# LCSL/nys-koop-lqr

Measured on AMD Instinct MI355X. Metric: Nyström-Koopman fits/sec (K_nm build + A,B,C solve), N=1e5 m=2000 d=384, higher is better.
Workload: dtype f64

## Files before the change

### include/nyskoop.h

```cpp
#ifndef NYSKOOP_H
#define NYSKOOP_H

#include <stdint.h>

#ifdef __cplusplus
extern "C" {
#endif

#define NK_ABI_VERSION 2

enum {
  NK_OK = 0,
  NK_ERR_BAD_ARG = -1,
  NK_ERR_HIP = -2,
  NK_ERR_NOT_SPD = -3,
  NK_ERR_OOM = -4,
  NK_ERR_NO_CONVERGENCE = -5,
  NK_ERR_NO_DEVICE = -6
};

enum { NK_KERNEL_RBF = 0, NK_KERNEL_MATERN52 = 1, NK_KERNEL_LINEAR = 2, NK_KERNEL_TPS = 3 };

typedef struct nk_kernel_desc {
  int32_t type;
  int32_t d;
  int32_t n_lengthscale;
  int32_t reserved;
  const double* lengthscale;
  double sigma0;
} nk_kernel_desc;

typedef struct nk_fit_stats {
  double ms_total;
  double ms_upload;
  double ms_kmat;
  double ms_gram;
  double ms_sqrt;
  double ms_solve;
  double ms_gram_kernel_avg;
  int32_t gram_kernel_launches;
  int32_t sqrt_iters;
  double sqrt_residual;
  double gram_flops;
  double kmat_pairs;
  int32_t rank_inner;
  int32_t rank_inner_rec;
  double pivot_ratio_inner;
  double pivot_ratio_inner_rec;
  int32_t refined;
  int32_t reserved_;
  double refine_ratio_inner;
  double refine_ratio_inner_rec;
} nk_fit_stats;

typedef struct nk_ctx nk_ctx;
typedef struct nk_model nk_model;

int nk_version(void);
const char* nk_last_error(void);
int nk_device_count(void);
int nk_create(int device, nk_ctx** out);
int nk_destroy(nk_ctx* ctx);
int nk_synchronize(nk_ctx* ctx);
void* nk_stream(nk_ctx* ctx);
int nk_set_kmat_mode(nk_ctx* ctx, int mode);
int nk_set_strict_spd(nk_ctx* ctx, int strict);
int nk_set_refine(nk_ctx* ctx, double pivot_ratio, int32_t steps);
#define NK_DTYPE_F64 0
#define NK_DTYPE_F32 1
int nk_set_compute_dtype(nk_ctx* ctx, int dtype);
int nk_wait_stream(nk_ctx* ctx, void* producer_stream);
int nk_group_create(int device, int size, nk_ctx** members);
typedef struct nk_cv_unit {
  const nk_kernel_desc* kernel;
  double gamma;
  double jitter;
  int32_t m;
  int32_t reserved;
  int64_t test_begin, test_end;
  const int64_t* landmark_rows;
} nk_cv_unit;
int nk_cv_grid(nk_ctx* const* members, int32_t n_members, const double* X, int64_t ldx, const double* Y, int64_t ldy,
               int64_t n, int32_t d, int32_t p, const nk_cv_unit* units, int32_t n_units, double* scores, int32_t* status);
typedef struct nk_spline_cv_unit {
  double gamma;
  int32_t m;
  int32_t reserved;
  int64_t test_begin, test_end;
  const double* centers;
} nk_spline_cv_unit;
int nk_spline_cv_grid(nk_ctx* const* members, int32_t n_members, const double* X, int64_t ldx, const double* Y,
                      int64_t ldy, int64_t n, int32_t d, int32_t p, const nk_spline_cv_unit* units, int32_t n_units,
                      double* scores, int32_t* status);
int nk_group_enter(nk_ctx* member);
int nk_group_leave(nk_ctx* member);
int nk_group_stats(nk_ctx* member, uint64_t* out4);
int nk_runtime_counters(uint64_t* out, int32_t n);
int nk_shutdown(void);

void* nk_host_alloc(uint64_t bytes);
void nk_host_free(void* ptr);

int nk_kernel_matrix(nk_ctx* ctx, const nk_kernel_desc* kd,
                     const double* A, int64_t lda, int64_t nA,
                     const double* B, int64_t ldb, int64_t nB,
                     double* out, int64_t ldo);

int nk_nystrom_fit(nk_ctx* ctx, const nk_kernel_desc* kd,
                   const double* X, int64_t ldx, const double* Y, int64_t ldy,
                   int64_t n, int32_t d, int32_t p,
                   const int64_t* row_ranges, int32_t n_ranges,
                   const double* Zin, int64_t ldzi, const double* Zout, int64_t ldzo, int32_t m,
                   double gamma, double jitter,
                   nk_model** model, nk_fit_stats* stats);

int nk_gram_doubles(int32_t m, int32_t d, int32_t p, int64_t* count);
int nk_nystrom_gram(nk_ctx* ctx, const nk_kernel_desc* kd,
                    const double* X, int64_t ldx, const double* Y, int64_t ldy,
                    int64_t n, int32_t d, int32_t p,
                    const int64_t* row_ranges, int32_t n_ranges,
                    const double* Zin, int64_t ldzi, const double* Zout, int64_t ldzo, int32_t m,
                    double* gram, nk_fit_stats* stats);
int nk_nystrom_solve(nk_ctx* ctx, const nk_kernel_desc* kd,
                     const double* Zin, int64_t ldzi, const double* Zout, int64_t ldzo, int32_t m, int32_t d, int32_t p,
                     const double* gram, int64_t n_total, double gamma, double jitter,
                     nk_model** model, nk_fit_stats* stats);

int nk_model_create(nk_ctx* ctx, const nk_kernel_desc* kd, const double* Zout, int64_t ldz,
                    int32_t m, int32_t d, int32_t p, double jitter,
                    const double* A, const double* B, const double* C, const double* W,
                    nk_model** model);
int nk_model_destroy(nk_model* model);

int nk_spline_fit(nk_ctx* ctx, const double* X, int64_t ldx, const double* Y, int64_t ldy, int64_t n, int32_t d, int32_t p,
                  const int64_t* row_ranges, int32_t n_ranges, const double* centers, int64_t ldc, int32_t m, double gamma,
                  nk_model** model, nk_fit_stats* stats);
int nk_spline_model_create(nk_ctx* ctx, const double* centers, int64_t ldc, int32_t m, int32_t d, int32_t p,
                           const double* A, const double* B, const double* C, const double* W, nk_model** model);

int nk_model_get(nk_ctx* ctx, const nk_model* model, char which, double* out, int64_t ldo);
int nk_model_dims(const nk_model* model, int32_t* m, int32_t* d, int32_t* p);
int nk_model_get_ops(nk_ctx* ctx, const nk_model* model, double* G, int64_t ldg, double* C, int64_t ldc, double* W,
                     int64_t ldw);
int nk_model_get_ops_async(nk_ctx* ctx, nk_model* model, double* G, int64_t ldg, double* C, int64_t ldc, double* W,
                           int64_t ldw);
int nk_model_wait(nk_model* model);

int nk_lift(nk_ctx* ctx, const nk_model* model, const double* Xq, int64_t ldx, int64_t nq,
            double* out, int64_t ldo);

int nk_predict(nk_ctx* ctx, const nk_model* model, const double* Xaug, int64_t ldx, int64_t nq,
               double* out, int64_t ldo);

int nk_score_neg_rmse(nk_ctx* ctx, const nk_model* model, const double* Xaug, int64_t ldx,
                      const double* Ytrue, int64_t ldy, int64_t nq, double* score);

int nk_rollout(nk_ctx* ctx, const nk_model* model, const double* x0, int64_t ldx0,
               const double* U, int32_t T, int32_t batch, double* out_x, double* out_z);

int nk_closed_loop(nk_ctx* ctx, const nk_model* model, const double* K, const double* phi0,
                   const double* phi_ref, int32_t steps, double* out_x, double* out_u);
int nk_closed_loop_batch(nk_ctx* ctx, const nk_model* model, const double* K, const double* phi0,
                         const double* phi_ref, int32_t steps, int32_t batch, double* out_x, double* out_u);
#define NK_PLANT_DUFFING 0
#define NK_PLANT_DOUBLE_INTEGRATOR 1
#define NK_PLANT_HJB 2
int nk_plant_step(int plant, double Ts, const double* x, const double* u, double* x_next);
int nk_plant_loop(nk_ctx* ctx, const nk_model* model, int plant, double Ts, const double* K, const double* x0,
                  const double* x_ref, int32_t steps, int32_t batch, double* out_x, double* out_u);
int nk_linear_rollout(nk_ctx* ctx, const double* A, const double* B, const double* C, int32_t m, int32_t d, int32_t p,
                      const double* z0, const double* U, int32_t T, int32_t batch, double* out_x, double* out_z);

int nk_gemm_f32(nk_ctx* ctx, int64_t M, int64_t N, int64_t K, const float* A, int64_t lda, const float* B, int64_t ldb,
                double* C, int64_t ldc);
int nk_gemm(nk_ctx* ctx, int transA, int transB, int64_t M, int64_t N, int64_t K, double alpha,
            const double* A, int64_t lda, const double* B, int64_t ldb, double beta, double* C, int64_t ldc);
int nk_sqrtm_spd(nk_ctx* ctx, const double* P, int64_t ldp, int32_t m, double* S, double* Sinv,
                 int32_t* iters, double* residual);
int nk_solve_spd(nk_ctx* ctx, const double* P, int64_t ldp, int32_t m, const double* R, int64_t ldr,
                 int32_t nrhs, double* X, int64_t ldxo);

int nk_bench_gram(nk_ctx* ctx, int64_t n, int32_t m, int32_t p, int32_t d, int32_t reps, double* ms_avg, double* flop);

#define NK_CHOL_FLOW_GIVEUP (-0x40000000)
int nk_chol_aug(nk_ctx* ctx, int32_t nsys, const double* const* P, const int64_t* ldp, const int32_t* m,
                const double* const* R, const int32_t* extra, double* const* L, double* const* X, int32_t* failed,
                double* piv_ratio);

#ifdef __cplusplus
}
#endif
#endif
```

### nys_koop_lqr_amd/_lib.py

```python
import atexit
import ctypes as C
import os
import sys
import threading

import numpy as np

_HERE = os.path.dirname(os.path.abspath(__file__))

NK_KERNEL_RBF, NK_KERNEL_MATERN52, NK_KERNEL_LINEAR, NK_KERNEL_TPS = 0, 1, 2, 3
NK_PLANT_DUFFING, NK_PLANT_DOUBLE_INTEGRATOR, NK_PLANT_HJB = 0, 1, 2
NK_OK = 0
_ERR_NAMES = {-1: "NK_ERR_BAD_ARG", -2: "NK_ERR_HIP", -3: "NK_ERR_NOT_SPD", -4: "NK_ERR_OOM",
              -5: "NK_ERR_NO_CONVERGENCE", -6: "NK_ERR_NO_DEVICE"}


class NyskoopError(RuntimeError):
    def __init__(self, code, msg):
        super().__init__(f"{_ERR_NAMES.get(code, code)}: {msg}")
        self.code = code


class KernelDesc(C.Structure):
    _fields_ = [("type", C.c_int32), ("d", C.c_int32), ("n_lengthscale", C.c_int32), ("reserved", C.c_int32),
                ("lengthscale", C.POINTER(C.c_double)), ("sigma0", C.c_double)]


class CvUnit(C.Structure):
    _fields_ = [("kernel", C.POINTER(KernelDesc)), ("gamma", C.c_double), ("jitter", C.c_double), ("m", C.c_int32),
                ("reserved", C.c_int32), ("test_begin", C.c_int64), ("test_end", C.c_int64),
                ("landmark_rows", C.POINTER(C.c_int64))]


class SplineCvUnit(C.Structure):
    _fields_ = [("gamma", C.c_double), ("m", C.c_int32), ("reserved", C.c_int32), ("test_begin", C.c_int64),
                ("test_end", C.c_int64), ("centers", C.POINTER(C.c_double))]


class FitStats(C.Structure):
    _fields_ = [("ms_total", C.c_double), ("ms_upload", C.c_double), ("ms_kmat", C.c_double),
                ("ms_gram", C.c_double), ("ms_sqrt", C.c_double), ("ms_solve", C.c_double),
                ("ms_gram_kernel_avg", C.c_double), ("gram_kernel_launches", C.c_int32),
                ("sqrt_iters", C.c_int32), ("sqrt_residual", C.c_double), ("gram_flops", C.c_double),
                ("kmat_pairs", C.c_double), ("rank_inner", C.c_int32), ("rank_inner_rec", C.c_int32),
                ("pivot_ratio_inner", C.c_double), ("pivot_ratio_inner_rec", C.c_double), ("refined", C.c_int32),
                ("reserved_", C.c_int32), ("refine_ratio_inner", C.c_double), ("refine_ratio_inner_rec", C.c_double)]

    def as_dict(self):
        return {k: getattr(self, k) for k, _ in self._fields_}


_P = C.c_void_p
_I64 = C.c_int64
_I32 = C.c_int32
_D = C.c_double

SIGNATURES = {
    "nk_version": (C.c_int, []),
    "nk_last_error": (C.c_char_p, []),
    "nk_device_count": (C.c_int, []),
    "nk_create": (C.c_int, [C.c_int, C.POINTER(_P)]),
    "nk_destroy": (C.c_int, [_P]),
    "nk_synchronize": (C.c_int, [_P]),
    "nk_stream": (_P, [_P]),
    "nk_set_kmat_mode": (C.c_int, [_P, C.c_int]),
    "nk_set_strict_spd": (C.c_int, [_P, C.c_int]),
    "nk_set_refine": (C.c_int, [_P, C.c_double, C.c_int32]),
    "nk_wait_stream": (C.c_int, [_P, _P]),
    "nk_shutdown": (C.c_int, []),
    "nk_group_create": (C.c_int, [C.c_int, C.c_int, C.POINTER(_P)]),
    "nk_group_enter": (C.c_int, [_P]),
    "nk_group_leave": (C.c_int, [_P]),
    "nk_set_compute_dtype": (C.c_int, [_P, C.c_int]),
    "nk_group_stats": (C.c_int, [_P, C.POINTER(C.c_uint64)]),
    "nk_runtime_counters": (C.c_int, [C.POINTER(C.c_uint64), C.c_int32]),
    "nk_cv_grid": (C.c_int, [C.POINTER(_P), _I32, _P, _I64, _P, _I64, _I64, _I32, _I32, C.POINTER(CvUnit), _I32,
                             C.POINTER(_D), C.POINTER(_I32)]),
    "nk_spline_cv_grid": (C.c_int, [C.POINTER(_P), _I32, _P, _I64, _P, _I64, _I64, _I32, _I32, C.POINTER(SplineCvUnit),
                                    _I32, C.POINTER(_D), C.POINTER(_I32)]),
    "nk_host_alloc": (_P, [C.c_uint64]),
    "nk_host_free": (None, [_P]),
    "nk_kernel_matrix": (C.c_int, [_P, C.POINTER(KernelDesc), _P, _I64, _I64, _P, _I64, _I64, _P, _I64]),
    "nk_nystrom_fit": (C.c_int, [_P, C.POINTER(KernelDesc), _P, _I64, _P, _I64, _I64, _I32, _I32,
                                 C.POINTER(_I64), _I32, _P, _I64, _P, _I64, _I32, _D, _D,
                                 C.POINTER(_P), C.POINTER(FitStats)]),
    "nk_gram_doubles": (C.c_int, [_I32, _I32, _I32, C.POINTER(_I64)]),
    "nk_nystrom_gram": (C.c_int, [_P, C.POINTER(KernelDesc), _P, _I64, _P, _I64, _I64, _I32, _I32,
                                  C.POINTER(_I64), _I32, _P, _I64, _P, _I64, _I32, _P, C.POINTER(FitStats)]),
    "nk_nystrom_solve": (C.c_int, [_P, C.POINTER(KernelDesc), _P, _I64, _P, _I64, _I32, _I32, _I32, _P, _I64, _D, _D,
                                   C.POINTER(_P), C.POINTER(FitStats)]),
    "nk_model_create": (C.c_int, [_P, C.POINTER(KernelDesc), _P, _I64, _I32, _I32, _I32, _D, _P, _P, _P, _P,
                                  C.POINTER(_P)]),
    "nk_spline_fit": (C.c_int, [_P, _P, _I64, _P, _I64, _I64, _I32, _I32, C.POINTER(_I64), _I32, _P, _I64, _I32, _D,
                                C.POINTER(_P), C.POINTER(FitStats)]),
    "nk_spline_model_create": (C.c_int, [_P, _P, _I64, _I32, _I32, _I32, _P, _P, _P, _P, C.POINTER(_P)]),
    "nk_model_destroy": (C.c_int, [_P]),
    "nk_model_get": (C.c_int, [_P, _P, C.c_char, _P, _I64]),
    "nk_model_dims": (C.c_int, [_P, C.POINTER(_I32), C.POINTER(_I32), C.POINTER(_I32)]),
    "nk_model_get_ops": (C.c_int, [_P, _P, _P, _I64, _P, _I64, _P, _I64]),
    "nk_model_get_ops_async": (C.c_int, [_P, _P, _P, _I64, _P, _I64, _P, _I64]),
    "nk_model_wait": (C.c_int, [_P]),
    "nk_lift": (C.c_int, [_P, _P, _P, _I64, _I64, _P, _I64]),
    "nk_predict": (C.c_int, [_P, _P, _P, _I64, _I64, _P, _I64]),
    "nk_score_neg_rmse": (C.c_int, [_P, _P, _P, _I64, _P, _I64, _I64, C.POINTER(_D)]),
    "nk_rollout": (C.c_int, [_P, _P, _P, _I64, _P, _I32, _I32, _P, _P]),
    "nk_closed_loop": (C.c_int, [_P, _P, _P, _P, _P, _I32, _P, _P]),
    "nk_closed_loop_batch": (C.c_int, [_P, _P, _P, _P, _P, _I32, _I32, _P, _P]),
    "nk_plant_step": (C.c_int, [C.c_int, _D, _P, _P, _P]),
    "nk_plant_loop": (C.c_int, [_P, _P, C.c_int, _D, _P, _P, _P, _I32, _I32, _P, _P]),
    "nk_linear_rollout": (C.c_int, [_P, _P, _P, _P, _I32, _I32, _I32, _P, _P, _I32, _I32, _P, _P]),
    "nk_gemm_f32": (C.c_int, [_P, _I64, _I64, _I64, _P, _I64, _P, _I64, _P, _I64]),
    "nk_gemm": (C.c_int, [_P, C.c_int, C.c_int, _I64, _I64, _I64, _D, _P, _I64, _P, _I64, _D, _P, _I64]),
    "nk_sqrtm_spd": (C.c_int, [_P, _P, _I64, _I32, _P, _P, C.POINTER(_I32), C.POINTER(_D)]),
    "nk_solve_spd": (C.c_int, [_P, _P, _I64, _I32, _P, _I64, _I32, _P, _I64]),
    "nk_bench_gram": (C.c_int, [_P, _I64, _I32, _I32, _I32, _I32, C.POINTER(_D), C.POINTER(_D)]),
    "nk_chol_aug": (C.c_int, [_P, _I32, _P, _P, _P, _P, _P, _P, _P, _P, _P]),
}

_lib = None
_lib_lock = threading.Lock()


def library_path():
    return os.environ.get("NYSKOOP_LIB", os.path.join(_HERE, "libnyskoop.so"))


def load_library():
    global _lib
    with _lib_lock:
        if _lib is None:
            path = library_path()
            if not os.path.exists(path):
                raise NyskoopError(-6, f"{path} not found: build it with `python -c 'import __graft_entry__ as g; "
                                       f"g.build()'` or `make -C nys_koop_lqr_amd/csrc` (there is no CPU fallback)")
            if os.environ.get("NYSKOOP_PRELOAD_TORCH", "1") == "1" and "torch" not in sys.modules:
                try:
                    import torch
                except Exception:
                    pass
            lib = C.CDLL(path)
            for name, (res, args) in SIGNATURES.items():
                fn = getattr(lib, name)
                fn.restype = res
                fn.argtypes = args
            _lib = lib
            atexit.register(shutdown)
    return _lib


def shutdown():
    lib = _lib
    if lib is None:
        return
    with _pools_lock:
        pools = list(_pools.values())
        _pools.clear()
        lpools = list(_lockstep_pools.values())
        _lockstep_pools.clear()
    for pool in pools:
        pool.shutdown(wait=True)
    for pool in lpools:
        pool.close()
    _PinnedBlock.drain()
    lib.nk_shutdown()


def check(rc):
    if rc != NK_OK:
        raise NyskoopError(rc, load_library().nk_last_error().decode("utf-8", "replace"))


def runtime_counters():
    v = (C.c_uint64 * 5)()
    check(load_library().nk_runtime_counters(v, 5))
    return dict(chain_giveups=int(v[0]), jacobi_giveups=int(v[1]), rank_truncated_fits=int(v[2]), sqrt_retries=int(v[3]),
                refined_fits=int(v[4]))


def torch_if_cuda():
    try:
        import torch
    except Exception:
        return None
    try:
        return torch if torch.cuda.is_available() else None
    except Exception:
        return None


class Mat:

    def __init__(self, obj, rows=None, cols=None):
        if hasattr(obj, "data_ptr") and hasattr(obj, "stride"):
            if str(getattr(obj, "dtype", "")).split(".")[-1] not in ("float64", "double"):
                raise TypeError("device tensors must be float64")
            if obj.dim() != 2 or (obj.shape[1] > 1 and obj.stride(1) != 1):
                raise ValueError("device tensors must be 2-D with unit inner stride")
            self.owner, self.ptr, self.ld = obj, obj.data_ptr(), int(obj.stride(0))
            self.shape = (int(obj.shape[0]), int(obj.shape[1]))
        else:
            a = np.asarray(obj, dtype=np.float64)
            if a.ndim == 1:
                a = a.reshape(1, -1)
            if a.ndim != 2:
                raise ValueError("expected a 2-D array")
            if a.shape[1] > 0 and a.shape[0] > 0 and (a.strides[1] != 8 or a.strides[0] % 8 or a.strides[0] < 8 * a.shape[1]):
                a = np.ascontiguousarray(a)
            self.owner, self.ptr = a, a.ctypes.data
            self.ld = a.strides[0] // 8 if a.shape[0] > 1 else max(a.shape[1], 1)
            self.shape = a.shape
        if self.shape[0] <= 1:
            self.ld = max(self.ld, self.shape[1], 1)
        if rows is not None and self.shape[0] != rows or cols is not None and self.shape[1] != cols:
            raise ValueError(f"expected a {rows} x {cols} matrix, got {self.shape}")


class Context:

    def __init__(self, device=0, handle=None):
        self.lib = load_library()
        if handle is None:
            handle = _P()
            check(self.lib.nk_create(int(device), C.byref(handle)))
        self.handle = handle
        self.device = int(device)

    def enter(self):
        check(self.lib.nk_group_enter(self.handle))

    def leave(self):
        check(self.lib.nk_group_leave(self.handle))

    def close(self):
        if getattr(self, "handle", None):
            self.lib.nk_destroy(self.handle)
# ... 268 lines not shown
```

### nys_koop_lqr_amd/csrc/nk_api.hip

```cpp
#include "nk_common.h"
#include "nk_plant.h"

#include <cmath>
#include <cstdarg>
#include <cstdio>
#include <cstring>
#include <chrono>
#include <cstdlib>
#include <algorithm>
#include <condition_variable>
#include <functional>
#include <mutex>
#include <set>
#include <thread>

namespace nk {

static thread_local std::string g_err;

void set_error(const char* fmt, ...) {
  char buf[1024];
  va_list ap;
  va_start(ap, fmt);
  vsnprintf(buf, sizeof(buf), fmt, ap);
// ... 197 lines not shown
    if (g_pool[i].device == device && g_pool[i].bytes == bytes) {
      double* p = g_pool[i].ptr;
      g_pool.erase(g_pool.begin() + i);
      return p;
    }
  return nullptr;
}
static void pool_give(int device, size_t bytes, double* ptr) {
  {
    std::lock_guard<std::mutex> lk(g_pool_mu);
    if (g_pool.size() < 512) {
      g_pool.push_back(ModelBuf{device, bytes, ptr});
      return;
    }
  }
  (void)hipSetDevice(device);
  (void)hipFree(ptr);
}
static void pool_drain() {
  std::lock_guard<std::mutex> lk(g_pool_mu);
  for (auto& b : g_pool) {
    (void)hipSetDevice(b.device);
    (void)hipFree(b.ptr);
  }
  g_pool.clear();
}

static int model_alloc(nk_ctx* ctx, int m, int d, int p, nk_model** out, int kind = NK_MODEL_NYSTROM) {
  nk_model* mdl = new nk_model();
  mdl->device = ctx->device;
  mdl->m = m; mdl->d = d; mdl->p = p;
  mdl->kind = kind;
  const size_t mp = (size_t)m + p;
  const size_t nS = kind == NK_MODEL_SPLINE ? 0 : 2 * (size_t)m * m;
  const size_t total = (size_t)m * mp  + (size_t)d * m  + (size_t)d * mp  + nS +
                       (size_t)m * d  + (size_t)d  + 64;
  mdl->bytes = total * sizeof(double);
  mdl->buf = pool_take(ctx->device, mdl->bytes);
  if (!mdl->buf) {
    hipError_t e = hipMalloc(reinterpret_cast<void**>(&mdl->buf), mdl->bytes);
    if (e != hipSuccess) {
      (void)hipGetLastError();
      delete mdl;
      set_error("model allocation of %zu bytes failed: %s", total * sizeof(double), hipGetErrorString(e));
      return NK_ERR_OOM;
    }
  }
  double* q = mdl->buf;
  auto take = [&](size_t cnt) { double* r = q; q += (cnt + 1) & ~(size_t)1; return r; };
  mdl->A = take((size_t)m * mp);
  mdl->B = mdl->A + m;
  mdl->C = take((size_t)d * m);
  mdl->W = take((size_t)d * mp);
  if (kind != NK_MODEL_SPLINE) {
    mdl->S = take((size_t)m * m);
    mdl->Sinv = take((size_t)m * m);
  }
  mdl->Z = take((size_t)m * d);
  mdl->winv = take((size_t)d);
  {
    std::lock_guard<std::mutex> lk(g_reg_mu);
    g_models.insert(mdl);
  }
  *out = mdl;
  return NK_OK;
}

static int lift_device(nk_ctx* ctx, const nk_model* mdl, const double* Xq, int64_t ldx, int64_t nq, double* out,
                       int64_t ldo) {
  const int m = mdl->m;
  if (mdl->kind == NK_MODEL_SPLINE)
    return launch_kmat(ctx, mdl->ktype, Xq, ldx, nq, mdl->Z, mdl->d, m, mdl->d, mdl->winv, mdl->sigma0, out, ldo);
  const int64_t chunk = 32768;
  const ArenaMark mk = arena_mark(ctx);
  double* Kq = nullptr;
  NK_TRY(arena_alloc_t(ctx, (size_t)(nq < chunk ? nq : chunk) * m, &Kq));
  for (int64_t r0 = 0; r0 < nq; r0 += chunk) {
    const int64_t len = nq - r0 < chunk ? nq - r0 : chunk;
    NK_TRY(launch_kmat(ctx, mdl->ktype, Xq + r0 * ldx, ldx, len, mdl->Z, mdl->d, m, mdl->d, mdl->winv, mdl->sigma0, Kq,
                       m));
    NK_TRY(launch_gemm(ctx, false, false, len, m, m, 1.0, Kq, m, mdl->Sinv, m, 0.0, out + r0 * ldo, ldo));
  }
  arena_release(ctx, mk);
  return NK_OK;
}

static int predict_device(nk_ctx* ctx, const nk_model* mdl, const double* Xaug, int64_t ldx, int64_t nq, double* out,
                          int64_t ldo) {
  const int m = mdl->m, d = mdl->d, p = mdl->p;
  const int64_t chunk = 32768;
  const ArenaMark mk = arena_mark(ctx);
  double* phi = nullptr;
  NK_TRY(arena_alloc_t(ctx, (size_t)(nq < chunk ? nq : chunk) * m, &phi));
  for (int64_t r0 = 0; r0 < nq; r0 += chunk) {
    const int64_t len = nq - r0 < chunk ? nq - r0 : chunk;
    NK_TRY(lift_device(ctx, mdl, Xaug + r0 * ldx, ldx, len, phi, m));
    NK_TRY(launch_gemm(ctx, false, true, len, d, m, 1.0, phi, m, mdl->W, m + p, 0.0, out + r0 * ldo, ldo));
    if (p > 0)
      NK_TRY(launch_gemm(ctx, false, true, len, d, p, 1.0, Xaug + r0 * ldx + d, ldx, mdl->W + m, m + p, 1.0,
                         out + r0 * ldo, ldo));
  }
  arena_release(ctx, mk);
  return NK_OK;
}

struct HostTrace {
  bool on;
  std::chrono::steady_clock::time_point t0, last;
  HostTrace() : on(getenv("NYSKOOP_TRACE") != nullptr) { t0 = last = std::chrono::steady_clock::now(); }
  void mark(const char* what) {
    if (!on) return;
    auto now = std::chrono::steady_clock::now();
    fprintf(stderr, "[nk trace] %-28s +%8.3f ms (total %8.3f)\n", what,
            std::chrono::duration<double, std::milli>(now - last).count(),
            std::chrono::duration<double, std::milli>(now - t0).count());
    last = now;
  }
};

static float ev_ms(nk_ctx* ctx, int a, int b) {
  float ms = 0.f;
  (void)hipEventElapsedTime(&ms, ctx->ev[a], ctx->ev[b]);
  return ms;
}

}

using namespace nk;

extern "C" {

int nk_version(void) { return NK_ABI_VERSION; }

const char* nk_last_error(void) { return g_err.c_str(); }

int nk_device_count(void) {
  int n = 0;
  if (hipGetDeviceCount(&n) != hipSuccess) {
    (void)hipGetLastError();
    return 0;
  }
  return n;
}

int nk_create(int device, nk_ctx** out) {
  NK_REQUIRE(out != nullptr, "nk_create: null output pointer");
  *out = nullptr;
  int n = nk_device_count();
  if (n <= 0) {
    set_error("no HIP device visible: libnyskoop has no CPU fallback");
    return NK_ERR_NO_DEVICE;
  }
  NK_REQUIRE(device >= 0 && device < n, "nk_create: device %d out of range (0..%d)", device, n - 1);
  NK_HIP(hipSetDevice(device));
  hipDeviceProp_t prop;
  NK_HIP(hipGetDeviceProperties(&prop, device));
  if (strncmp(prop.gcnArchName, "gfx950", 6) != 0) {
    set_error("device %d is %s; libnyskoop is built for gfx950 (MI355X) only", device, prop.gcnArchName);
    return NK_ERR_NO_DEVICE;
  }
  nk_ctx* ctx = new nk_ctx();
  ctx->device = device;
  ctx->num_cu = prop.multiProcessorCount;
  int prio_lo = 0, prio_hi = 0;
  NK_HIP(hipDeviceGetStreamPriorityRange(&prio_lo, &prio_hi));
  const int prio_mid = (prio_lo - prio_hi >= 2) ? (prio_lo + prio_hi) / 2 : prio_hi;
  NK_HIP(hipStreamCreateWithPriority(&ctx->stream_main, hipStreamNonBlocking, prio_mid));
  NK_HIP(hipStreamCreateWithPriority(&ctx->stream_side, hipStreamNonBlocking, prio_lo));
  NK_HIP(hipStreamCreateWithPriority(&ctx->stream_prep, hipStreamNonBlocking, prio_hi));
  NK_HIP(hipStreamCreateWithFlags(&ctx->stream_copy, hipStreamNonBlocking));
  NK_HIP(hipStreamCreateWithPriority(&ctx->stream_la[0], hipStreamNonBlocking, prio_hi));
  NK_HIP(hipStreamCreateWithPriority(&ctx->stream_la[1], hipStreamNonBlocking, prio_mid));
  for (int q = 0; q < 2; ++q)
    for (int i = 0; i < 4; ++i) NK_HIP(hipEventCreateWithFlags(&ctx->ev_la[q][i], hipEventDisableTiming));
  ctx->stream = ctx->stream_main;
  ctx->cur_arena = &ctx->arena;
  NK_HIP(hipEventCreateWithFlags(&ctx->ev_fork, hipEventDisableTiming));
  NK_HIP(hipEventCreateWithFlags(&ctx->ev_join, hipEventDisableTiming));
  NK_HIP(hipEventCreateWithFlags(&ctx->ev_chain, hipEventDisableTiming));
  NK_HIP(hipMalloc(reinterpret_cast<void**>(&ctx->d_info), 256));
  ctx->d_piv = reinterpret_cast<unsigned long long*>(ctx->d_info + 16);
  NK_HIP(hipMalloc(reinterpret_cast<void**>(&ctx->d_scalars), 64 * sizeof(double)));
  NK_HIP(hipHostMalloc(reinterpret_cast<void**>(&ctx->h_scalars), 64 * sizeof(double), hipHostMallocMapped | hipHostMallocCoherent));
  NK_HIP(hipHostMalloc(reinterpret_cast<void**>(&ctx->h_info), 256, hipHostMallocMapped | hipHostMallocCoherent));
  ctx->h_piv = reinterpret_cast<unsigned long long*>(ctx->h_info + 16);
  for (int i = 0; i < 16; ++i) NK_HIP(hipEventCreate(&ctx->ev[i]));
  NK_HIP(hipEventCreateWithFlags(&ctx->ev_ext, hipEventDisableTiming));
  for (int i = 0; i < 8; ++i) NK_HIP(hipEventCreateWithFlags(&ctx->ev_up[i], hipEventDisableTiming));
  const char* km = getenv("NYSKOOP_KMAT");
  ctx->kmat_mode = (km && strcmp(km, "direct") == 0) ? 1 : 0;
  const char* st = getenv("NYSKOOP_STRICT_SPD");
  ctx->strict_spd = (st && atoi(st) != 0) ? 1 : 0;
  if (const char* rp = getenv("NYSKOOP_REFINE_PIVOT")) ctx->refine_pivot = atof(rp);
  if (const char* rs = getenv("NYSKOOP_REFINE_STEPS")) ctx->refine_steps = std::max(0, atoi(rs));
  {
    std::lock_guard<std::mutex> lk(g_reg_mu);
    g_ctxs.insert(ctx);
  }
  *out = ctx;
  return NK_OK;
}

static void destroy_ctx_unregistered(nk_ctx* ctx) {
  (void)hipSetDevice(ctx->device);
  if (tl_ctx == ctx) tl_ctx = nullptr;
  group_detach(ctx);
  (void)hipStreamSynchronize(ctx->stream_main);
  (void)hipStreamSynchronize(ctx->stream_side);
  (void)hipStreamSynchronize(ctx->stream_prep);
  (void)hipStreamSynchronize(ctx->stream_copy);
  for (int q = 0; q < 2; ++q) {
    if (ctx->stream_la[q]) { (void)hipStreamSynchronize(ctx->stream_la[q]); (void)hipStreamDestroy(ctx->stream_la[q]); }
    for (int i = 0; i < 4; ++i) if (ctx->ev_la[q][i]) (void)hipEventDestroy(ctx->ev_la[q][i]);
  }
  for (auto& c : ctx->arena.chunks) (void)hipFree(c.base);
  for (auto& c : ctx->arena_side.chunks) (void)hipFree(c.base);
  (void)hipEventDestroy(ctx->ev_fork);
  (void)hipEventDestroy(ctx->ev_join);
  if (ctx->ev_chain) (void)hipEventDestroy(ctx->ev_chain);
  if (ctx->ev_ext) (void)hipEventDestroy(ctx->ev_ext);
  for (int i = 0; i < 8; ++i) if (ctx->ev_up[i]) (void)hipEventDestroy(ctx->ev_up[i]);
  (void)hipStreamDestroy(ctx->stream_side);
  (void)hipStreamDestroy(ctx->stream_prep);
  (void)hipStreamDestroy(ctx->stream_copy);
  (void)hipFree(ctx->d_info);
  for (int i = 0; i < 2; ++i) if (ctx->d_flow[i]) (void)hipFree(ctx->d_flow[i]);
  (void)hipFree(ctx->d_scalars);
  if (ctx->d_zeros) (void)hipFree(ctx->d_zeros);
  if (ctx->h_stage) (void)hipHostFree(ctx->h_stage);
  (void)hipHostFree(ctx->h_scalars);
  (void)hipHostFree(ctx->h_info);
  for (int i = 0; i < 16; ++i) (void)hipEventDestroy(ctx->ev[i]);
  (void)hipStreamDestroy(ctx->stream_main);
  delete ctx;
}

int nk_destroy(nk_ctx* ctx) {
  if (!ctx) return NK_OK;
  {
    std::lock_guard<std::mutex> lk(g_reg_mu);
    if (g_ctxs.erase(ctx) == 0) return NK_OK;
  }
  destroy_ctx_unregistered(ctx);
  return NK_OK;
}

static int model_wait_unchecked(nk_model* mdl);
static void destroy_model_unregistered(nk_model* model, bool to_pool) {
  (void)model_wait_unchecked(model);
  if (to_pool) {
    pool_give(model->device, model->bytes, model->buf);
  } else {
    (void)hipSetDevice(model->device);
    (void)hipFree(model->buf);
  }
  delete model;
}

int nk_shutdown(void) {
  tl_ctx = nullptr;
  std::set<nk_ctx*> ctxs;
  std::set<nk_model*> models;
  std::set<void*> blocks;
  {
    std::lock_guard<std::mutex> lk(g_reg_mu);
    ctxs.swap(g_ctxs);
    models.swap(g_models);
    blocks.swap(g_host_blocks);
  }
  for (nk_ctx* c : ctxs) {
    (void)hipSetDevice(c->device);
    (void)hipStreamSynchronize(c->stream_main);
    (void)hipStreamSynchronize(c->stream_side);
    (void)hipStreamSynchronize(c->stream_prep);
    (void)hipStreamSynchronize(c->stream_copy);
  }
  for (nk_model* m : models) destroy_model_unregistered(m, false);
  for (nk_ctx* c : ctxs) destroy_ctx_unregistered(c);
  pool_drain();
  for (void* b : blocks) (void)hipHostFree(b);
  return NK_OK;
}

int nk_set_compute_dtype(nk_ctx* ctx, int dtype) {
  NK_REQUIRE(ctx != nullptr && (dtype == NK_DTYPE_F64 || dtype == NK_DTYPE_F32), "nk_set_compute_dtype: bad argument");
  ctx->compute_f32 = dtype == NK_DTYPE_F32 ? 1 : 0;
  return NK_OK;
}

int nk_set_strict_spd(nk_ctx* ctx, int strict) {
  NK_REQUIRE(ctx != nullptr && strict >= 0 && strict <= 2, "nk_set_strict_spd: bad argument");
  ctx->strict_spd = strict;
  return NK_OK;
}

int nk_set_refine(nk_ctx* ctx, double pivot_ratio, int32_t steps) {
  NK_REQUIRE(ctx != nullptr && pivot_ratio >= 0.0 && pivot_ratio <= 1.0 && steps >= 0 && steps <= 8, "nk_set_refine: bad argument");
  ctx->refine_pivot = pivot_ratio;
  ctx->refine_steps = steps;
  return NK_OK;
}

int nk_wait_stream(nk_ctx* ctx, void* producer_stream) {
  NK_REQUIRE(ctx != nullptr, "nk_wait_stream: null context");
  NK_HIP(hipSetDevice(ctx->device));
  if (ctx->group) {
    hipError_t e = real_stream_sync(reinterpret_cast<hipStream_t>(producer_stream));
    if (e != hipSuccess) { set_error("synchronising the producer stream failed: %s", hipGetErrorString(e)); return NK_ERR_HIP; }
    return NK_OK;
  }
  NK_HIP(hipEventRecord(ctx->ev_ext, reinterpret_cast<hipStream_t>(producer_stream)));
  NK_HIP(hipStreamWaitEvent(ctx->stream_main, ctx->ev_ext, 0));
  NK_HIP(hipStreamWaitEvent(ctx->stream_side, ctx->ev_ext, 0));
  NK_HIP(hipStreamWaitEvent(ctx->stream_prep, ctx->ev_ext, 0));
  NK_HIP(hipStreamWaitEvent(ctx->stream_copy, ctx->ev_ext, 0));
  return NK_OK;
}

int nk_group_create(int device, int size, nk_ctx** out) {
  NK_REQUIRE(out != nullptr && size >= 1 && size <= 256, "nk_group_create: bad argument");
  for (int i = 0; i < size; ++i) out[i] = nullptr;
  for (int i = 0; i < size; ++i) {
    int rc = nk_create(device, &out[i]);
    if (rc != NK_OK) {
      for (int j = 0; j < i; ++j) { nk_destroy(out[j]); out[j] = nullptr; }
      return rc;
    }
  }
  nk_group* g = group_new(device, size);
  if (!g) {
    for (int i = 0; i < size; ++i) { nk_destroy(out[i]); out[i] = nullptr; }
    set_error("nk_group_create: could not create the shared stream / argument table");
    return NK_ERR_HIP;
  }
  for (int i = 0; i < size; ++i) group_attach(g, i, out[i]);
  return NK_OK;
}

int nk_group_enter(nk_ctx* ctx) {
  NK_REQUIRE(ctx != nullptr, "nk_group_enter: null context");
  return group_enter(ctx);
}

// ... 125 lines not shown
  for (int k = 0; k < B; ++k) set_phase(members[k], k, 1);
  run_units(all, true);
  for (int k = 0; k < B; ++k) set_phase(members[k], k, 0);
  const auto t_mid = std::chrono::steady_clock::now();
  if (!deferred.empty()) {
    std::sort(deferred.begin(), deferred.end());
    for (int k = 0; k < B; ++k) set_phase(members[k], k, 2);
    run_units(deferred, false);
    for (int k = 0; k < B; ++k) set_phase(members[k], k, 0);
  }
  if (cv_trace)
    fprintf(stderr, "[nyskoop] %s: %d units in %.3f s, %zu rank-deficient units again in %.3f s (%d members)\n", what, n_units,
            std::chrono::duration<double>(t_mid - t_start).count(), deferred.size(),
            std::chrono::duration<double>(std::chrono::steady_clock::now() - t_mid).count(), B);
  return NK_OK;
}

int nk_cv_grid(nk_ctx* const* members, int32_t n_members, const double* X, int64_t ldx, const double* Y, int64_t ldy,
               int64_t n, int32_t d, int32_t p, const nk_cv_unit* units, int32_t n_units, double* scores, int32_t* status) {
  NK_REQUIRE(members && n_members >= 1 && X && Y && units && scores, "nk_cv_grid: null argument");
  NK_REQUIRE(n > 0 && d > 0 && p >= 0 && n_units >= 0 && ldx >= d + p && ldy >= d, "nk_cv_grid: bad sizes");
  for (int k = 0; k < n_members; ++k) NK_REQUIRE(members[k] != nullptr, "nk_cv_grid: null member context");
  for (int u = 0; u < n_units; ++u) {
    const nk_cv_unit& cu = units[u];
    NK_REQUIRE(cu.kernel && cu.landmark_rows && cu.m > 0, "nk_cv_grid: unit %d: null kernel / landmarks", u);
    NK_REQUIRE(0 <= cu.test_begin && cu.test_begin < cu.test_end && cu.test_end <= n, "nk_cv_grid: unit %d: bad test fold", u);
    for (int j = 0; j < cu.m; ++j)
      NK_REQUIRE(cu.landmark_rows[j] >= 0 && cu.landmark_rows[j] < n, "nk_cv_grid: unit %d: landmark row out of range", u);
  }
  auto fit_score = [&](nk_ctx* ctx, int u, const CvData& dt, std::vector<double>& Z, double* sc) -> int {
    const nk_cv_unit& cu = units[u];
    Z.resize((size_t)cu.m * d);
    for (int j = 0; j < cu.m; ++j) memcpy(&Z[(size_t)j * d], dt.Yh + cu.landmark_rows[j] * dt.ldyh, (size_t)d * 8);
    const int64_t rr[4] = {0, cu.test_begin, cu.test_end, n};
    nk_model* mdl = nullptr;
    int rc = nk_nystrom_fit(ctx, cu.kernel, dt.Xd, dt.ldxd, dt.Yd, dt.ldyd, n, d, p, rr, 2, nullptr, 0, Z.data(), d, cu.m,
                            cu.gamma, cu.jitter, &mdl, nullptr);
    if (rc == NK_OK)
      rc = nk_score_neg_rmse(ctx, mdl, dt.Xd + cu.test_begin * dt.ldxd, dt.ldxd, dt.Yd + cu.test_begin * dt.ldyd, dt.ldyd,
                             cu.test_end - cu.test_begin, sc);
    if (mdl) nk_model_destroy(mdl);
    return rc;
  };
  std::vector<int> saved_strict((size_t)n_members);
  for (int k = 0; k < n_members; ++k) saved_strict[(size_t)k] = members[k]->strict_spd;
  auto set_phase = [&](nk_ctx* ctx, int k, int phase) {
    ctx->strict_spd = phase == 1 ? 1 : (phase == 2 ? 0 : saved_strict[(size_t)k]);
  };
  return cv_grid_run("cv_grid", members, n_members, X, ldx, Y, ldy, n, d, p, n_units, true, fit_score, set_phase, scores,
                     status);
}

int nk_spline_cv_grid(nk_ctx* const* members, int32_t n_members, const double* X, int64_t ldx, const double* Y, int64_t ldy,
                      int64_t n, int32_t d, int32_t p, const nk_spline_cv_unit* units, int32_t n_units, double* scores,
                      int32_t* status) {
  NK_REQUIRE(members && n_members >= 1 && X && Y && units && scores, "nk_spline_cv_grid: null argument");
  NK_REQUIRE(n > 0 && d > 0 && p >= 0 && n_units >= 0 && ldx >= d + p && ldy >= d, "nk_spline_cv_grid: bad sizes");
  for (int k = 0; k < n_members; ++k) NK_REQUIRE(members[k] != nullptr, "nk_spline_cv_grid: null member context");
  for (int u = 0; u < n_units; ++u) {
    const nk_spline_cv_unit& cu = units[u];
    NK_REQUIRE(cu.centers && cu.m > 0, "nk_spline_cv_grid: unit %d: null centres / m <= 0", u);
    NK_REQUIRE(!is_device_ptr(cu.centers), "nk_spline_cv_grid: unit %d: centres must be a host pointer", u);
    NK_REQUIRE(0 <= cu.test_begin && cu.test_begin < cu.test_end && cu.test_end <= n,
               "nk_spline_cv_grid: unit %d: bad test fold", u);
  }
  auto fit_score = [&](nk_ctx* ctx, int u, const CvData& dt, std::vector<double>&, double* sc) -> int {
    const nk_spline_cv_unit& cu = units[u];
    const int64_t rr[4] = {0, cu.test_begin, cu.test_end, n};
    nk_model* mdl = nullptr;
    int rc = nk_spline_fit(ctx, dt.Xd, dt.ldxd, dt.Yd, dt.ldyd, n, d, p, rr, 2, cu.centers, d, cu.m, cu.gamma, &mdl, nullptr);
    if (rc == NK_OK)
      rc = nk_score_neg_rmse(ctx, mdl, dt.Xd + cu.test_begin * dt.ldxd, dt.ldxd, dt.Yd + cu.test_begin * dt.ldyd, dt.ldyd,
                             cu.test_end - cu.test_begin, sc);
    if (mdl) nk_model_destroy(mdl);
    return rc;
  };
  auto set_phase = [&](nk_ctx* ctx, int, int phase) { ctx->spline_defer_svd = phase == 1; };
  return cv_grid_run("spline_cv_grid", members, n_members, X, ldx, Y, ldy, n, d, p, n_units, false, fit_score, set_phase,
                     scores, status);
}

int nk_synchronize(nk_ctx* ctx) {
  NK_REQUIRE(ctx != nullptr, "null context");
  tl_ctx = ctx;
  NK_HIP(hipStreamSynchronize(ctx->stream));
  return NK_OK;
}

void* nk_stream(nk_ctx* ctx) { return ctx ? reinterpret_cast<void*>(ctx->stream) : nullptr; }

void* nk_host_alloc(uint64_t bytes) {
  void* p = nullptr;
  if (hipHostMalloc(&p, bytes ? bytes : 1, hipHostMallocDefault) != hipSuccess) {
    (void)hipGetLastError();
    set_error("hipHostMalloc of %llu bytes failed", (unsigned long long)bytes);
    return nullptr;
  }
  std::lock_guard<std::mutex> lk(g_reg_mu);
  g_host_blocks.insert(p);
  return p;
}

void nk_host_free(void* ptr) {
  if (!ptr) return;
  {
    std::lock_guard<std::mutex> lk(g_reg_mu);
    if (g_host_blocks.erase(ptr) == 0) return;
  }
  (void)hipHostFree(ptr);
}

int nk_set_kmat_mode(nk_ctx* ctx, int mode) {
  NK_REQUIRE(ctx != nullptr && (mode == 0 || mode == 1), "nk_set_kmat_mode: bad argument");
  ctx->kmat_mode = mode;
  return NK_OK;
}

int nk_kernel_matrix(nk_ctx* ctx, const nk_kernel_desc* kd, const double* A, int64_t lda, int64_t nA, const double* B,
                     int64_t ldb, int64_t nB, double* out, int64_t ldo) {
  NK_TRY(check_ctx(ctx));
  NK_REQUIRE(kd && A && B && out, "nk_kernel_matrix: null argument");
  NK_REQUIRE(nA >= 0 && nB >= 0 && kd->d > 0, "nk_kernel_matrix: negative size");
  NK_REQUIRE(lda >= kd->d && ldb >= kd->d && ldo >= nB, "nk_kernel_matrix: leading dimension too small");
  if (nA == 0 || nB == 0) return NK_OK;
  const int d = kd->d;
  double* winv = nullptr;
  NK_TRY(arena_alloc_t(ctx, (size_t)d, &winv));
  NK_TRY(make_winv(ctx, kd, d, winv));
  MatIn a, b;
  NK_TRY(stage_in(ctx, A, lda, nA, d, &a));
  NK_TRY(stage_in(ctx, B, ldb, nB, d, &b));
  MatOut o;
  NK_TRY(stage_out(ctx, out, ldo, nA, nB, &o));
  if (kd->type == NK_KERNEL_TPS && ctx->kmat_mode == 0 && d >= 32 && nA >= 2 && nB >= 2) {
    const int64_t lta = (nA + 1) & ~(int64_t)1, ltb = (nB + 1) & ~(int64_t)1;
    double *center = nullptr, *At = nullptr, *sqa = nullptr, *Bt = nullptr, *sqb = nullptr;
    NK_TRY(arena_alloc_t(ctx, (size_t)d, &center));
    NK_TRY(arena_alloc_t(ctx, (size_t)d * lta, &At));
    NK_TRY(arena_alloc_t(ctx, (size_t)nA, &sqa));
    NK_TRY(arena_alloc_t(ctx, (size_t)d * ltb, &Bt));
    NK_TRY(arena_alloc_t(ctx, (size_t)nB, &sqb));
    NK_TRY(launch_colmean(ctx, b.ptr, b.ld, (int)nB, d, center));
    NK_TRY(prep_rows(ctx, a.ptr, a.ld, nA, d, winv, center, At, lta, sqa));
    NK_TRY(prep_rows(ctx, b.ptr, b.ld, nB, d, winv, center, Bt, ltb, sqb));
    NK_TRY(launch_kmat_gram(ctx, NK_KERNEL_TPS, At, lta, sqa, nA, Bt, ltb, sqb, nB, d, 0.0, o.dev, o.ld));
  } else {
    NK_TRY(launch_kmat(ctx, kd->type, a.ptr, a.ld, nA, b.ptr, b.ld, nB, d, winv, kd->sigma0, o.dev, o.ld));
  }
  NK_TRY(finish_out(ctx, o));
  NK_HIP(hipStreamSynchronize(ctx->stream));
  return NK_OK;
}

static inline size_t gram_block1(int m, int p) { return (((size_t)(2 * m + p) * (m + p)) + 1) & ~(size_t)1; }
static inline size_t gram_doubles(int m, int d, int p) { return gram_block1(m, p) + (size_t)(m + d) * m; }

enum { FIT_FULL = 0, FIT_GRAM = 1, FIT_SOLVE = 2 };

static int fit_impl(nk_ctx* ctx, const nk_kernel_desc* kd, const double* X, int64_t ldx, const double* Y, int64_t ldy,
                    int64_t n, int32_t d, int32_t p, const int64_t* row_ranges, int32_t n_ranges, const double* Zin,
                    int64_t ldzi, const double* Zout, int64_t ldzo, int32_t m, double gamma, double jitter,
                    nk_model** model, nk_fit_stats* stats, int mode, double* gram_io) {
  HostTrace tr;
  NK_TRY(check_ctx(ctx));
  tr.mark("check_ctx/arena_reset");
  NK_REQUIRE(kd && Zout, "nk_nystrom_fit: null argument");
  NK_REQUIRE(mode == FIT_SOLVE || (X && Y), "nk_nystrom_fit: null data pointer");
  NK_REQUIRE(mode == FIT_GRAM || model != nullptr, "nk_nystrom_fit: null model pointer");
  NK_REQUIRE(mode == FIT_FULL || gram_io != nullptr, "nk_nystrom_gram/solve: null accumulator");
  NK_REQUIRE(n > 0 && d > 0 && p >= 0 && m > 0, "nk_nystrom_fit: sizes must be positive (n=%lld d=%d p=%d m=%d)",
             (long long)n, d, p, m);
  NK_REQUIRE(mode == FIT_SOLVE || (ldx >= d + p && ldy >= d), "nk_nystrom_fit: leading dimension too small");
  NK_REQUIRE(ldzo >= d, "nk_nystrom_fit: leading dimension too small");
  NK_REQUIRE(std::isfinite(gamma) && std::isfinite(jitter), "nk_nystrom_fit: gamma/jitter not finite");
  NK_REQUIRE(kd->type != NK_KERNEL_TPS, "nk_nystrom_fit: the thin-plate spline has no Nystrom fit (nk_spline_fit)");
  if (model) *model = nullptr;
  std::vector<int64_t> rng;
  if (mode != FIT_SOLVE && row_ranges && n_ranges > 0) {
    for (int i = 0; i < n_ranges; ++i) {
      const int64_t b = row_ranges[2 * i], e = row_ranges[2 * i + 1];
      NK_REQUIRE(0 <= b && b <= e && e <= n, "nk_nystrom_fit: row range %d = [%lld,%lld) outside [0,%lld)", i,
                 (long long)b, (long long)e, (long long)n);
      if (e > b) { rng.push_back(b); rng.push_back(e); }
    }
  } else {
    rng.push_back(0); rng.push_back(n);
  }
  int64_t n_eff = 0;
  for (size_t i = 0; i < rng.size(); i += 2) n_eff += rng[i + 1] - rng[i];
  NK_REQUIRE(n_eff > 0, "nk_nystrom_fit: no training rows selected");
  const bool same_centers = (Zin == nullptr) || (Zin == Zout && ldzi == ldzo);
  const int mp = m + p;
  const double gamma_n = gamma * (double)n_eff;

  nk_model* mdl = nullptr;
  NK_TRY(model_alloc(ctx, m, d, p, &mdl));
  struct Guard {
    nk_ctx* c;
    nk_model* m;
    ~Guard() {
      if (m) {
        (void)hipStreamSynchronize(c->stream_main);
        (void)hipStreamSynchronize(c->stream_side);
        (void)hipStreamSynchronize(c->stream_prep);
        (void)hipStreamSynchronize(c->stream_la[0]);
        (void)hipStreamSynchronize(c->stream_la[1]);
        nk_model_destroy(m);
      }
    }
  } guard{ctx, mdl};
  mdl->ktype = kd->type; mdl->sigma0 = kd->sigma0; mdl->jitter = jitter;

  tr.mark("validate + model_alloc");
  hipEvent_t* ev = ctx->ev;
  NK_HIP(hipEventRecord(ev[0], ctx->stream));
  NK_TRY(make_winv(ctx, kd, d, mdl->winv));
  MatIn x, y, zi, zo;
  int host_passes = 1;
  if (mode != FIT_SOLVE) {
    const char* e = getenv("NYSKOOP_HOST_PASSES");
    const int want = e ? atoi(e) : 6;
    if (want > 1 && rng.size() == 2 && !ctx_recording(ctx) && (double)n_eff * (2.0 * d + p) * 8.0 >= 64e6 &&
        !is_device_ptr(X) && !is_device_ptr(Y))
      host_passes = want > 8 ? 8 : want;
  }
  if (mode != FIT_SOLVE && host_passes > 1) {
    x.ld = (d + p + 1) & ~(int64_t)1;
    y.ld = (d + 1) & ~(int64_t)1;
    double *xd = nullptr, *yd = nullptr;
    NK_TRY(arena_alloc_t(ctx, (size_t)n * x.ld, &xd));
    NK_TRY(arena_alloc_t(ctx, (size_t)n * y.ld, &yd));
    x.ptr = xd; y.ptr = yd; x.staged = y.staged = true;
  } else if (mode != FIT_SOLVE) {
    NK_TRY(stage_in(ctx, X, ldx, n, d + p, &x));
    NK_TRY(stage_in(ctx, Y, ldy, n, d, &y));
  }
  if (mode != FIT_SOLVE && rng.size() > 2 && (double)n_eff * (2.0 * d + p) * 8.0 <= 256e6) {
    const int64_t ldxg = (d + p + 1) & ~(int64_t)1, ldyg = (d + 1) & ~(int64_t)1;
    double *xg = nullptr, *yg = nullptr;
    NK_TRY(arena_alloc_t(ctx, (size_t)n_eff * ldxg, &xg));
    NK_TRY(arena_alloc_t(ctx, (size_t)n_eff * ldyg, &yg));
    int64_t o = 0;
    for (size_t i = 0; i < rng.size(); i += 2) {
      const int64_t b = rng[i], len = rng[i + 1] - rng[i];
      NK_TRY(launch_copy2d(ctx, x.ptr + b * x.ld, x.ld, xg + o * ldxg, ldxg, len, d + p));
      NK_TRY(launch_copy2d(ctx, y.ptr + b * y.ld, y.ld, yg + o * ldyg, ldyg, len, d));
      o += len;
    }
    x.ptr = xg; x.ld = ldxg; y.ptr = yg; y.ld = ldyg;
    rng.assign({(int64_t)0, n_eff});
  }
  NK_TRY(stage_in(ctx, Zout, ldzo, m, d, &zo));
  if (same_centers) zi = zo; else NK_TRY(stage_in(ctx, Zin, ldzi, m, d, &zi));
  NK_TRY(launch_copy2d(ctx, zo.ptr, zo.ld, mdl->Z, d, m, d));
  NK_HIP(hipEventRecord(ev[1], ctx->stream));
  tr.mark("staging issued");

  double *Kmm = nullptr, *Kj = nullptr, *Kj_in = nullptr, *Kxo = nullptr;
  bool landmarks_aside = false;
  if (mode != FIT_GRAM) {
  NK_TRY(arena_alloc_t(ctx, (size_t)m * m, &Kmm));
  NK_TRY(arena_alloc_t(ctx, (size_t)m * m, &Kj));
  if (same_centers) {
    Kj_in = Kj;
    Kxo = Kmm;
  } else {
    NK_TRY(arena_alloc_t(ctx, (size_t)m * m, &Kj_in));
    NK_TRY(arena_alloc_t(ctx, (size_t)m * m, &Kxo));
  }
  {
    const char* la = getenv("NYSKOOP_LANDMARKS_ASIDE");
    landmarks_aside = mode == FIT_FULL && n_eff >= 20000 && m >= 1024 && !ctx_recording(ctx) && !(la && la[0] == '0');
  }
  {
    hipStream_t s0 = ctx->stream;
    if (landmarks_aside) {
      NK_HIP(hipEventRecord(ev[12], ctx->stream));
      ctx->stream = ctx->stream_prep;
      NK_HIP(hipStreamWaitEvent(ctx->stream, ev[12], 0));
    }
    int rc_l = launch_kmat(ctx, kd->type, zo.ptr, zo.ld, m, zo.ptr, zo.ld, m, d, mdl->winv, kd->sigma0, Kmm, m);
    if (rc_l == NK_OK) rc_l = launch_copy2d(ctx, Kmm, m, Kj, m, m, m);
    if (rc_l == NK_OK) rc_l = launch_add_diag(ctx, Kj, m, m, jitter);
    if (rc_l == NK_OK && !same_centers) {
      rc_l = launch_kmat(ctx, kd->type, zi.ptr, zi.ld, m, zi.ptr, zi.ld, m, d, mdl->winv, kd->sigma0, Kj_in, m);
      if (rc_l == NK_OK) rc_l = launch_add_diag(ctx, Kj_in, m, m, jitter);
      if (rc_l == NK_OK) rc_l = launch_kmat(ctx, kd->type, zi.ptr, zi.ld, m, zo.ptr, zo.ld, m, d, mdl->winv, kd->sigma0, Kxo, m);
    }
    const hipError_t he = rc_l == NK_OK ? hipEventRecord(ev[8], ctx->stream) : hipSuccess;
    ctx->stream = s0;
    NK_TRY(rc_l);
    NK_HIP(he);
  }
  }
  double *G1 = nullptr, *G2 = nullptr, *G3 = nullptr, *G4 = nullptr;
  const int64_t ldd = d + (d & 1);
  NK_TRY(arena_alloc_t(ctx, gram_doubles(m, d, p), &G1));
  G2 = G1 + (size_t)mp * mp;
  G3 = G1 + gram_block1(m, p);
  G4 = G3 + (size_t)m * m;
  float ms_gram_kernel = 0.f;
  int gram_launches = 0;
  bool gram_deferred = false;
  const bool timed = stats != nullptr;
  SqrtPlan splan;
  int it = 0;
// ... 1640 lines not shown
```

### nys_koop_lqr_amd/csrc/nk_common.h

```cpp
#pragma once
#include <hip/hip_runtime.h>
#include <stdint.h>
#include <stddef.h>
#include <string>
#include <vector>

#include "nyskoop.h"
#include "nk_lockstep.h"

namespace nk {

void set_error(const char* fmt, ...);

#define NK_HIP(call)                                                                         \
  do {                                                                                       \
    hipError_t e_ = (call);                                                                  \
    if (e_ != hipSuccess) {                                                                  \
      nk::set_error("%s failed: %s (%s:%d)", #call, hipGetErrorString(e_), __FILE__, __LINE__); \
      return e_ == hipErrorOutOfMemory ? NK_ERR_OOM : NK_ERR_HIP;                            \
    }                                                                                        \
  } while (0)

#define NK_TRY(call)            \
  do {                          \
    int rc_ = (call);           \
    if (rc_ != NK_OK) return rc_; \
  } while (0)

#define NK_REQUIRE(cond, ...)     \
  do {                            \
    if (!(cond)) {                \
      nk::set_error(__VA_ARGS__); \
      return NK_ERR_BAD_ARG;      \
    }                             \
  } while (0)

struct ArenaChunk {
  char* base = nullptr;
  size_t cap = 0;
  size_t off = 0;
};
struct Arena {
  std::vector<ArenaChunk> chunks;
  int cur = 0;
};
struct ArenaMark {
  int chunk;
  size_t off;
};

}

struct nk_member_state;
struct nk_ctx {
  int device = 0;
  hipStream_t stream = nullptr;
  hipStream_t stream_main = nullptr;
  hipStream_t stream_side = nullptr;
  hipStream_t stream_copy = nullptr;
  hipStream_t stream_prep = nullptr;
  nk::Arena arena;
  nk::Arena arena_side;
  nk::Arena* cur_arena = nullptr;
  hipStream_t stream_la[2] = {nullptr, nullptr};
  hipEvent_t ev_la[2][4] = {};
  int compute_f32 = 0;
  hipEvent_t ev_fork = nullptr, ev_join = nullptr, ev_chain = nullptr;
  int* d_info = nullptr;
  unsigned long long* d_piv = nullptr;
  unsigned long long* h_piv = nullptr;
  double* d_scalars = nullptr;
  double* h_scalars = nullptr;
  int* h_info = nullptr;
  double* d_zeros = nullptr;
  hipEvent_t ev[16];
  int num_cu = 256;
  int kmat_mode = 0;
  double refine_pivot = 0.0;
  int refine_steps = 2;
  int strict_spd = 0;
  hipEvent_t ev_ext = nullptr;
  hipEvent_t ev_up[8] = {};
  nk_group* group = nullptr;
  nk_member_state* gstate = nullptr;
  int* d_flow[2] = {nullptr, nullptr};
  size_t flow_words[2] = {0, 0};
  bool spline_defer_svd = false;
  bool chol_flow_off = false;
  double* h_stage = nullptr;
  size_t h_stage_bytes = 0;
};

enum { NK_MODEL_NYSTROM = 0, NK_MODEL_SPLINE = 1 };
struct nk_model {
  int device = 0;
  int32_t m = 0, d = 0, p = 0;
  int32_t ktype = 0;
  double sigma0 = 0.0;
  double jitter = 0.0;
  double* buf = nullptr;
  size_t bytes = 0;
  double *A = nullptr, *B = nullptr, *C = nullptr, *W = nullptr, *S = nullptr, *Sinv = nullptr, *Z = nullptr,
         *winv = nullptr;
  bool has_ops = false;
  int32_t kind = 0;
  hipEvent_t ev_fetch = nullptr;
};

namespace nk {

struct SideScope {
  nk_ctx* c;
  hipStream_t s0;
  Arena* a0;
  explicit SideScope(nk_ctx* ctx, hipStream_t s = nullptr) : c(ctx), s0(ctx->stream), a0(ctx->cur_arena) {
    c->stream = s ? s : c->stream_side;
    c->cur_arena = &c->arena_side;
  }
  ~SideScope() {
    c->stream = s0;
    c->cur_arena = a0;
  }
};

struct ChainOnly {
  nk_ctx* c;
  bool b0;
  explicit ChainOnly(nk_ctx* ctx) : c(ctx), b0(ctx->chol_flow_off) { c->chol_flow_off = true; }
  ~ChainOnly() { c->chol_flow_off = b0; }
};

inline int info_base(const nk_ctx* c) { return c->stream != c->stream_main ? 2 : 0; }

__device__ __forceinline__ double exp_nonpos_ca() {
  double ca = __longlong_as_double(0x3e5ade156a5dcb37LL);
  asm volatile("" : "+v"(ca));
  return ca;
}
__device__ __forceinline__ double exp_nonpos(double x, double ca_v) {
  const double k = __builtin_rint(x * __longlong_as_double(0x3ff71547652b82feLL));
  double r = __builtin_fma(__longlong_as_double((long long)0xbfe62e42fefa39efULL), k, x);
  r = __builtin_fma(__longlong_as_double((long long)0xbc7abc9e3b39803fULL), k, r);
  double p;
#define NK_EXP_STEP(c) asm("v_fma_f64 %0, %1, %2, %3" : "=v"(p) : "v"(r), "v"(p), "s"(c))
  asm("v_fma_f64 %0, %1, %2, %3" : "=v"(p) : "v"(r), "v"(ca_v), "s"(__longlong_as_double(0x3e928af3fca7ab0cLL)));
  NK_EXP_STEP(__longlong_as_double(0x3ec71dee623fde64LL));
  NK_EXP_STEP(__longlong_as_double(0x3efa01997c89e6b0LL));
  NK_EXP_STEP(__longlong_as_double(0x3f2a01a014761f6eLL));
  NK_EXP_STEP(__longlong_as_double(0x3f56c16c1852b7b0LL));
  NK_EXP_STEP(__longlong_as_double(0x3f81111111122322LL));
  NK_EXP_STEP(__longlong_as_double(0x3fa55555555502a1LL));
  NK_EXP_STEP(__longlong_as_double(0x3fc5555555555511LL));
  NK_EXP_STEP(__longlong_as_double(0x3fe000000000000bLL));
#undef NK_EXP_STEP
  p = __builtin_fma(r, p, 1.0);
  p = __builtin_fma(r, p, 1.0);
  return x < -1075.0 ? 0.0 : ldexp(p, (int)k);
}
__device__ __forceinline__ double exp_nonpos(double x) { return exp_nonpos(x, exp_nonpos_ca()); }

__host__ __device__ __forceinline__ double log_pos(double x) {
#pragma clang fp contract(off)
  const double ln2_hi = 6.93147180369123816490e-01, ln2_lo = 1.90821492927058770002e-10;
  const double Lg1 = 6.666666666666735130e-01, Lg2 = 3.999999999940941908e-01, Lg3 = 2.857142874366239149e-01,
               Lg4 = 2.222219843214978396e-01, Lg5 = 1.818357216161805012e-01, Lg6 = 1.531383769920937332e-01,
               Lg7 = 1.479819860511658591e-01;
  uint64_t bits;
  __builtin_memcpy(&bits, &x, 8);
  int32_t hx = (int32_t)(bits >> 32);
  int k = 0;
  if (hx < 0x00100000) {
    x *= 1.80143985094819840000e+16;
    k -= 54;
    __builtin_memcpy(&bits, &x, 8);
    hx = (int32_t)(bits >> 32);
  }
  k += (hx >> 20) - 1023;
  hx &= 0x000fffff;
  const int32_t i = (hx + 0x95f64) & 0x100000;
  bits = ((uint64_t)(uint32_t)(hx | (i ^ 0x3ff00000)) << 32) | (bits & 0xffffffffULL);
  __builtin_memcpy(&x, &bits, 8);
  k += i >> 20;
  const double f = x - 1.0;
  const double dk = (double)k;
  if ((0x000fffff & (2 + hx)) < 3) {
    if (f == 0.0) return k == 0 ? 0.0 : dk * ln2_hi + dk * ln2_lo;
    const double R = f * f * (0.5 - 0.33333333333333333 * f);
    return k == 0 ? f - R : dk * ln2_hi - ((R - dk * ln2_lo) - f);
  }
  const double s = f / (2.0 + f);
  const double z = s * s;
  const double w = z * z;
  const double t1 = w * (Lg2 + w * (Lg4 + w * Lg6));
  const double t2 = z * (Lg1 + w * (Lg3 + w * (Lg5 + w * Lg7)));
  const double R = t2 + t1;
  if (((hx - 0x6147a) | (0x6b851 - hx)) > 0) {
    const double hfsq = 0.5 * f * f;
    return k == 0 ? f - (hfsq - s * (hfsq + R)) : dk * ln2_hi - ((hfsq - (s * (hfsq + R) + dk * ln2_lo)) - f);
  }
  return k == 0 ? f - s * (f - R) : dk * ln2_hi - ((s * (f - R) - dk * ln2_lo) - f);
}
__host__ __device__ __forceinline__ double tps_value(double r2) {
#pragma clang fp contract(off)
  return r2 > 0.0 ? r2 * log_pos(sqrt(r2)) : 0.0;
}

nk_group* group_new(int device, int size);
void group_attach(nk_group* g, int slot, nk_ctx* c);
void group_detach(nk_ctx* c);
int group_enter(nk_ctx* c);
int group_leave(nk_ctx* c);
void group_stats(nk_ctx* c, uint64_t out[4]);
enum { CNT_CHAIN_GIVEUP = 0, CNT_JACOBI_GIVEUP = 1, CNT_RANK_TRUNCATED = 2, CNT_SQRT_RETRY = 3, CNT_REFINED = 4,
       CNT_CHOL_FLOW_GIVEUP = 5, CNT_CHOL_FLOW = 6, CNT_N = 7 };
void count_event(int which);
uint64_t read_counter(int which);
hipError_t real_stream_sync(hipStream_t s);
hipError_t real_event_sync(hipEvent_t e);

int arena_reset(nk_ctx* ctx);
ArenaMark arena_mark(nk_ctx* ctx);
void arena_release(nk_ctx* ctx, ArenaMark mk);
int arena_alloc(nk_ctx* ctx, size_t bytes, void** out);
template <typename T>
inline int arena_alloc_t(nk_ctx* ctx, size_t count, T** out) {
  return arena_alloc(ctx, count * sizeof(T), reinterpret_cast<void**>(out));
}
bool is_device_ptr(const void* p);

int launch_kmat(nk_ctx* ctx, int ktype, const double* A, int64_t lda, int64_t nA, const double* B, int64_t ldb,
                int64_t nB, int d, const double* winv, double sigma0, double* out, int64_t ldo);

enum { TRI_FULL = 0, TRI_UPPER_MIRROR = 1, TRI_LOWER = 2 };
struct GemmOpts {
  int tri = TRI_FULL;
  int splitk = 0;
};
int launch_gemm(nk_ctx* ctx, bool transA, bool transB, int64_t M, int64_t N, int64_t K, double alpha, const double* A,
                int64_t lda, const double* B, int64_t ldb, double beta, double* C, int64_t ldc,
                const GemmOpts& opts = GemmOpts(), float* ms_kernel = nullptr);

struct GemmCall {
  int64_t M = 0, N = 0, K = 0;
  double alpha = 1.0, beta = 0.0;
  const double* A = nullptr;
  const double* B = nullptr;
  double* C = nullptr;
  int64_t lda = 0, ldb = 0, ldc = 0;
  GemmOpts opts;
};
int launch_gemm_pair(nk_ctx* ctx, bool transA, bool transB, const GemmCall* calls, int ncalls);

struct TnSkip;
int launch_add_diag(nk_ctx* ctx, double* A, int64_t lda, int n, double v);
int launch_copy2d(nk_ctx* ctx, const double* src, int64_t lds, double* dst, int64_t ldd, int64_t rows, int64_t cols);
int launch_axpby2d(nk_ctx* ctx, double a, const double* X, int64_t ldx, double b, double* Y, int64_t ldy,
                   int64_t rows, int64_t cols);
int launch_scale_add_identity(nk_ctx* ctx, double a, const double* X, int64_t ldx, double c, double* Y, int64_t ldy,
                              int n, const TnSkip* skip = nullptr);
int launch_fill(nk_ctx* ctx, double* A, int64_t lda, int64_t rows, int64_t cols, double v);
int launch_frob_minus_identity(nk_ctx* ctx, const double* M, int64_t ldm, int n, double* d_out,
                               const TnSkip* skip = nullptr);
int launch_max_abs_rowsum(nk_ctx* ctx, const double* M, int64_t ldm, int n, double* d_out);
int launch_colsum_sqdiff(nk_ctx* ctx, const double* P, int64_t ldp, const double* Y, int64_t ldy, int64_t rows,
                         int cols, double* d_colsum);

int sqrtm_spd(nk_ctx* ctx, const double* P, int64_t ldp, int m, double* S, double* Sinv, int* iters, double* resid);
struct SqrtPlan {
  const double* P = nullptr;
  int64_t ldp = 0;
  int m = 0;
  double* W = nullptr;
  double* Linv = nullptr;
  double* X0 = nullptr;
  double* X0t = nullptr;
  double* d_sc = nullptr;
  ArenaMark mark{0, 0};
  bool deferred = false;
  int rc = 0, iters = 0, kmax = 0;
  double resid = 0.0;
  double lambda_min_hint = 0.0;
  bool early = false;
  int info_slot = 2;
  bool flow_gave_up = false;
  hipEvent_t pause_event = nullptr;
  int pause_step = -1;
};
constexpr int NK_SQRT_RETRY = 1;
int sqrtm_spd_coupled(nk_ctx* ctx, const double* P, int64_t ldp, int m, double* S, double* Sinv, int* iters, double* resid);
int sqrtm_prepare(nk_ctx* ctx, const double* P, int64_t ldp, int m, SqrtPlan* plan);
int sqrtm_finish(nk_ctx* ctx, SqrtPlan* plan, double* S, double* Sinv);
int sqrtm_verdict(nk_ctx* ctx, SqrtPlan* plan, int* iters, double* resid);
int cholesky_lower(nk_ctx* ctx, double* P, int64_t ldp, int m, double* Linv );
int cholesky_solve(nk_ctx* ctx, const double* L, int64_t ldl, int m, const double* Linv, double* R, int64_t ldr,
                   int nrhs);
struct CholSys {
  double* P = nullptr;
  int64_t ldp = 0;
  int m = 0;
  int extra = 0;
  bool backward = true;
  double* Linv = nullptr;
  double* pivlog = nullptr;
  double* R = nullptr;
  int64_t ldr = 0;
  int nrhs = 0;
};
int cholesky_lower_pair(nk_ctx* ctx, const CholSys* sys, int nsys);
int cholesky_lower_pair_async(nk_ctx* ctx, const CholSys* sys, int nsys);
int cholesky_check_pair(nk_ctx* ctx, const CholSys* sys, int nsys);
int cholesky_solve_pair(nk_ctx* ctx, const CholSys* sys, int nsys);
int cholesky_aug_pair_async(nk_ctx* ctx, const CholSys* sys, int nsys, hipEvent_t pause = nullptr, int pause_step = -1);
constexpr int CHOL_NB = 64;
constexpr int CHOL_WS = 2 * CHOL_NB * CHOL_NB + 8;
constexpr double CHOL_FIX_KAPPA = 8.0 * CHOL_NB;
inline int chol_fix_enabled() {
  const char* e = getenv("NYSKOOP_CHOL_FIX");
  return (e && e[0] == '0') ? 0 : ((e && e[0] == '2') ? 2 : 1);
}
bool launch_chol_trail_pair(nk_ctx* ctx, const GemmCall* calls, int ncalls, int* rc);
bool launch_chol_trail_potrf_pair(nk_ctx* ctx, const GemmCall* calls, int ncalls, const int* nb, double* const* Linv, int blk,
                                  double* const* plog, int* rc);
inline bool chol_fuse_enabled() {
  const char* e = getenv("NYSKOOP_CHOL_FUSE");
  return !(e && e[0] == '0');
}
bool chol_flow_enabled();
int cholesky_flow_pair(nk_ctx* ctx, const CholSys* sys, int nsys);
constexpr int CHOL_FLOW_GIVEUP = -0x40000000;
bool launch_chol_panel_pair(nk_ctx* ctx, const GemmCall* calls, int ncalls, int* rc);
int launch_trsm_right_lower_pair(nk_ctx* ctx, const CholSys* sys, int nsys);

struct PinvInfo {
  int rank = 0, sweeps = 0;
  bool converged = false;
  double sigma_max = 0.0, sigma_min_kept = 0.0, sigma_min = 0.0;
};
int pinv_right_divide(nk_ctx* ctx, const double* P, int64_t ldp, int m, const double* E, int64_t lde, int rows,
                      double* E_out, int64_t ldeo, double rcond, PinvInfo* info);
int cholesky_fail_flags(nk_ctx* ctx, const CholSys* sys, int nsys, int* failed , double* piv_ratio = nullptr);

int launch_lifted_step(nk_ctx* ctx, const double* G, int64_t ldg, int m, int mz, int pu, const double* z, int64_t zstride,
                       const double* u, int64_t ustride, const double* bias, double* out, int64_t ostride, int batch);

struct ChainArgs {
  const double* G = nullptr; int64_t ldg = 0; int m = 0, pu = 0;
  const double* z0 = nullptr; int64_t z0_stride = 0;
  bool lift = false;
  const double* x0 = nullptr; int64_t x0_stride = 0;
  const double* Zl = nullptr; int d = 0; const double* winv = nullptr; const double* Sinv = nullptr; int ktype = 0;
  double sigma0 = 0.0;
  const double* U = nullptr; int64_t u_stride = 0;
  const double* bias = nullptr; int64_t bias_stride = 0;
  double* Zall = nullptr; int64_t z_stride = 0;
  int T = 0, batch = 0;
};
int launch_ref_minus_traj(nk_ctx* ctx, const double* ref, int64_t ref_stride, const double* Phi, int64_t phi_stride,
                          double* D, int64_t d_stride, int steps, int m, int batch);
bool lifted_chain_ok(int m, int pu, int d_lift);
int launch_lifted_chain(nk_ctx* ctx, const ChainArgs& a);
bool lifted_chain_mw_ok(const nk_ctx* ctx, int m, int pu);
int chain_mw_workgroups(int m);
int chain_mw_group(int m, int batch);
int launch_lifted_chain_mw(nk_ctx* ctx, const ChainArgs& a);
int lifted_chain_mw_reset(nk_ctx* ctx);
int lifted_chain_mw_fetch_status(nk_ctx* ctx);
bool lifted_chain_mw_timed_out(nk_ctx* ctx, int* row, int* step, int* traj);
// ... 113 lines not shown
```

### nys_koop_lqr_amd/csrc/nk_gemm_tn.hip

```cpp
#include "nk_common.h"
#include "nk_tn_kstep.inc"
#include "nk_tn_shared.h"

#include <cstdlib>
#include <cstring>

namespace nk {

typedef double d4 __attribute__((ext_vector_type(4)));

constexpr int TBK = 16;
constexpr int TSTRIDE = 144;
constexpr int TSTAGE = 2 * TBK * TSTRIDE;
constexpr int TN_LDS_BYTES = 2 * TSTAGE * 8;

struct TnDev {
  const double* A;
  const double* B;
  int64_t lda, ldb;
  int M, N;
  int tiles_n;
  int tri;
  int ktrim;
  int tile_begin;
  double* C;
  int64_t ldc;
  double alpha, beta;
  double* Ct;
  int64_t ldct;
  const double* A_even;
  const double* B_even;
  double* Caff;
  double aff_a, aff_c;
};
struct TnParams {
  TnDev p[TN_MAXP];
  int nprob;
  int ntiles;
  int K, splitk, klen;
  int kmask;
  int use_asm;
  const double* zeros;
  double* slab;
  const double* skip_state;
  int skip_step;
  const double* select_state;
  const double* sqa;
  const double* sqb;
  double* out;
  int64_t ldo;
  int ktype;
  double sigma0sq;
};

__device__ __forceinline__ uint64_t uniform_u64(uint64_t v) {
  return ((uint64_t)(uint32_t)__builtin_amdgcn_readfirstlane((uint32_t)(v >> 32)) << 32) |
         (uint64_t)(uint32_t)__builtin_amdgcn_readfirstlane((uint32_t)v);
}
__device__ __forceinline__ void dma_row(const double* row_base, uint32_t lane_off_bytes, uint32_t lds_addr) {
  const uint64_t rbu = uniform_u64((uint64_t)(uintptr_t)row_base);
  asm volatile("s_mov_b32 m0, %2\n\ts_nop 0\n\tglobal_load_lds_dwordx4 %0, %1"
               :
               : "v"(lane_off_bytes), "s"(rbu), "s"((uint32_t)__builtin_amdgcn_readfirstlane(lds_addr))
               : "m0");
}
__device__ __forceinline__ void dma_wait_all() { asm volatile("s_waitcnt vmcnt(0)" ::: "memory"); }

template <int EPI>
__device__ __forceinline__ void tn_body(const TnParams& P) {
  extern __shared__ __attribute__((aligned(16))) double smem[];
  const int split = blockIdx.x % P.splitk;
  const int gt = blockIdx.x / P.splitk;
  int pi = 0;
#pragma unroll
  for (int q = 1; q < TN_MAXP; ++q)
    if (q < P.nprob && gt >= P.p[q].tile_begin) pi = q;
  const TnDev pr = P.p[pi];
  int tm, tn;
  if (EPI >= 1) {
    const int xcd = blockIdx.x & 7, i = blockIdx.x >> 3;
    const int cols = (pr.tiles_n - xcd + 7) >> 3;
    if (cols <= 0) return;
    tm = i / cols;
    tn = xcd + 8 * (i - tm * cols);
    if (tm * TBM >= pr.M) return;
  } else {
    tn_tile_coords(gt - pr.tile_begin, pr.tri, pr.tiles_n, pr.M, tm, tn);
  }
  const int lane = threadIdx.x & 63;
  const int wave = __builtin_amdgcn_readfirstlane(threadIdx.x >> 6);
  if (EPI == 0 && P.skip_state != nullptr) {
    const double f = P.skip_state[0];
    if (f != 0.0 && f <= (double)P.skip_step) return;
  }
  const double* opA = pr.A;
  const double* opB = pr.B;
  if (EPI == 0 && P.select_state != nullptr && (((int)P.select_state[0]) & 1) == 0) {
    if (pr.A_even) opA = pr.A_even;
    if (pr.B_even) opB = pr.B_even;
  }
  int kbeg = split * P.klen;
  int kend = min(P.K, kbeg + P.klen);
  if (pr.ktrim == KTRIM_B_UPPER) kend = min(kend, (tn + 1) * TBM);
  if (pr.ktrim == KTRIM_A_LOWER) kbeg = max(kbeg, tm * TBM);
  const int ktiles = kend > kbeg ? (kend - kbeg + TBK - 1) / TBK : 0;

  const uint32_t offa = (uint32_t)min(tm * TBM + lane * 2, (pr.M - 1) & ~1) * 8u;
  const uint32_t offb = (uint32_t)min(tn * TBM + lane * 2, (pr.N - 1) & ~1) * 8u;
  const uint32_t offz = (uint32_t)lane * 16u;

  const uint32_t lds0 = (uint32_t)(uintptr_t)smem;
  auto issue = [&](int kt, int stage) {
    const uint32_t sa = lds0 + (uint32_t)(stage * TSTAGE) * 8u;
    const uint32_t sb = sa + (uint32_t)(TBK * TSTRIDE) * 8u;
    const int k0 = kbeg + kt * TBK;
    if (k0 + TBK <= kend) {
#pragma unroll
      for (int q = 0; q < 4; ++q) {
        const int r = wave + 4 * q;
        dma_row(opA + (int64_t)((k0 + r) & P.kmask) * pr.lda, offa, sa + (uint32_t)(r * TSTRIDE) * 8u);
        dma_row(opB + (int64_t)((k0 + r) & P.kmask) * pr.ldb, offb, sb + (uint32_t)(r * TSTRIDE) * 8u);
      }
    } else {
#pragma unroll
      for (int q = 0; q < 4; ++q) {
        const int r = wave + 4 * q;
        const int k = k0 + r;
        if (k < kend) {
          dma_row(opA + (int64_t)k * pr.lda, offa, sa + (uint32_t)(r * TSTRIDE) * 8u);
          dma_row(opB + (int64_t)k * pr.ldb, offb, sb + (uint32_t)(r * TSTRIDE) * 8u);
        } else {
          dma_row(P.zeros, offz, sa + (uint32_t)(r * TSTRIDE) * 8u);
          dma_row(P.zeros, offz, sb + (uint32_t)(r * TSTRIDE) * 8u);
        }
      }
    }
  };

  d4 acc[4][4];
#pragma unroll
  for (int i = 0; i < 4; ++i)
#pragma unroll
    for (int j = 0; j < 4; ++j) acc[i][j] = d4{0.0, 0.0, 0.0, 0.0};

  const int wm = wave >> 1, wn = wave & 1;
  const int r16 = lane & 15, g4 = lane >> 4;

  auto frag = [&](int stage, int ks, double (&a)[4], double (&b)[4]) {
    const double* a_base = smem + stage * TSTAGE + wm * 64 + r16 + (ks * 4 + g4) * TSTRIDE;
    const double* b_base = a_base + TBK * TSTRIDE + (wn - wm) * 64;
#pragma unroll
    for (int i = 0; i < 4; ++i) a[i] = a_base[i * 16];
#pragma unroll
    for (int j = 0; j < 4; ++j) b[j] = b_base[j * 16];
  };
  auto mma = [&](const double (&a)[4], const double (&b)[4]) {
#pragma unroll
    for (int i = 0; i < 4; ++i)
#pragma unroll
      for (int j = 0; j < 4; ++j)
        acc[i][j] = __builtin_amdgcn_mfma_f64_16x16x4f64(a[i], b[j], acc[i][j], 0, 0, 0);
  };
  double a0[4], b0[4], a1[4], b1[4];
  if (ktiles > 0) {
    issue(0, 0);
    dma_wait_all();
    __syncthreads();
    frag(0, 0, a0, b0);
  }
  const uint32_t ard0 = lds0 + (uint32_t)(wm * 64 + r16 + g4 * TSTRIDE) * 8u;
  const uint32_t brd0 = lds0 + (uint32_t)(TBK * TSTRIDE + wn * 64 + r16 + g4 * TSTRIDE) * 8u;
  constexpr uint32_t STAGE_B = (uint32_t)TSTAGE * 8u;
  const uint32_t stra = (uint32_t)__builtin_amdgcn_readfirstlane((uint32_t)(pr.lda * 32));
  const uint32_t strb = (uint32_t)__builtin_amdgcn_readfirstlane((uint32_t)(pr.ldb * 32));
#define NK_TN_ACC_OPERANDS                                                                                             \
  [c00] "+v"(acc[0][0]), [c01] "+v"(acc[0][1]), [c02] "+v"(acc[0][2]), [c03] "+v"(acc[0][3]), [c10] "+v"(acc[1][0]),   \
      [c11] "+v"(acc[1][1]), [c12] "+v"(acc[1][2]), [c13] "+v"(acc[1][3]), [c20] "+v"(acc[2][0]),                      \
      [c21] "+v"(acc[2][1]), [c22] "+v"(acc[2][2]), [c23] "+v"(acc[2][3]), [c30] "+v"(acc[3][0]),                      \
      [c31] "+v"(acc[3][1]), [c32] "+v"(acc[3][2]), [c33] "+v"(acc[3][3]), [a00] "+v"(a0[0]), [a01] "+v"(a0[1]),       \
      [a02] "+v"(a0[2]), [a03] "+v"(a0[3]), [b00] "+v"(b0[0]), [b01] "+v"(b0[1]), [b02] "+v"(b0[2]), [b03] "+v"(b0[3]), \
      [a10] "=&v"(a1[0]), [a11] "=&v"(a1[1]), [a12] "=&v"(a1[2]), [a13] "=&v"(a1[3]), [b10] "=&v"(b1[0]),              \
      [b11] "=&v"(b1[1]), [b12] "=&v"(b1[2]), [b13] "=&v"(b1[3])
#define NK_TN_IN_OPERANDS                                                                                             \
  [ard0] "v"(ard0), [brd0] "v"(brd0), [ard1] "v"(ard1), [brd1] "v"(brd1), [voa] "v"(offa), [vob] "v"(offb),           \
      [rowa] "s"(rowa), [rowb] "s"(rowb), [stra] "s"(stra), [strb] "s"(strb), [dst0] "s"(dst0), [dst1] "s"(dst1)
#define NK_TN_CLOBBERS "memory", "m0", "scc", "s92", "s93", "s94", "s95"
  const int nfull = (kend - kbeg) / TBK;
  int kt_start = 0;
  if (P.kmask == -1 && P.use_asm && nfull >= 1) {
    const uint32_t dst0 = (uint32_t)__builtin_amdgcn_readfirstlane(lds0 + (uint32_t)(wave * TSTRIDE) * 8u);
    const uint32_t dst1 = dst0 + STAGE_B;
    const uint32_t ard1 = ard0 + STAGE_B, brd1 = brd0 + STAGE_B;
    const int steady = nfull - 1;
    uint32_t cnt = (uint32_t)__builtin_amdgcn_readfirstlane((uint32_t)(steady / 2));
    const uint32_t flags =
        (uint32_t)__builtin_amdgcn_readfirstlane((uint32_t)((steady & 1) | (nfull == ktiles ? 2 : 0)));
    kt_start = 2 * (int)cnt + (int)(flags & 1) + (int)(flags >> 1);
    const uint64_t rowa = uniform_u64((uint64_t)(uintptr_t)(opA + (int64_t)(kbeg + TBK + wave) * pr.lda));
    const uint64_t rowb = uniform_u64((uint64_t)(uintptr_t)(opB + (int64_t)(kbeg + TBK + wave) * pr.ldb));
    if (kt_start > 0)
      asm volatile(NK_TN_KSTEPS_ASM
                   : NK_TN_ACC_OPERANDS, [cnt] "+s"(cnt)
                   : NK_TN_IN_OPERANDS, [flags] "s"(flags)
                   : NK_TN_CLOBBERS);
  }
  for (int kt = kt_start; kt < ktiles; ++kt) {
    const int st = kt & 1;
    const bool more = kt + 1 < ktiles;
    frag(st, 1, a1, b1);
    if (more) issue(kt + 1, st ^ 1);
    mma(a0, b0);
    __builtin_amdgcn_sched_barrier(0);
    frag(st, 2, a0, b0);
    __builtin_amdgcn_sched_barrier(0);
    mma(a1, b1);
    __builtin_amdgcn_sched_barrier(0);
    frag(st, 3, a1, b1);
    __builtin_amdgcn_sched_barrier(0);
    mma(a0, b0);
    __builtin_amdgcn_sched_barrier(0);
    dma_wait_all();
    __syncthreads();
    if (more) frag(st ^ 1, 0, a0, b0);
    __builtin_amdgcn_sched_barrier(0);
    mma(a1, b1);
    __builtin_amdgcn_sched_barrier(0);
  }

  if (EPI == 0 && P.splitk == 1) {
    const bool mirror = pr.tri == TRI_UPPER_MIRROR && tm != tn;
#pragma unroll
    for (int i = 0; i < 4; ++i)
#pragma unroll
      for (int j = 0; j < 4; ++j)
#pragma unroll
        for (int reg = 0; reg < 4; ++reg) {
          const int row = tm * TBM + wm * 64 + i * 16 + g4 + 4 * reg;
          const int col = tn * TBM + wn * 64 + j * 16 + r16;
          if (row < pr.M && col < pr.N) {
            double v = pr.alpha * acc[i][j][reg];
            if (pr.beta != 0.0) v += pr.beta * pr.C[(int64_t)row * pr.ldc + col];
            pr.C[(int64_t)row * pr.ldc + col] = v;
            if (mirror) pr.C[(int64_t)col * pr.ldc + row] = v;
            if (pr.Ct) pr.Ct[(int64_t)col * pr.ldct + row] = v;
            if (pr.Caff) {
              pr.Caff[(int64_t)row * pr.ldc + col] = pr.aff_a * v + (row == col ? pr.aff_c : 0.0);
              if (mirror) pr.Caff[(int64_t)col * pr.ldc + row] = pr.aff_a * v;
            }
          }
        }
  } else if (EPI == 0) {
    double* out = P.slab + ((int64_t)gt * P.splitk + split) * (TBM * TBM);
#pragma unroll
    for (int i = 0; i < 4; ++i)
#pragma unroll
      for (int j = 0; j < 4; ++j)
#pragma unroll
        for (int reg = 0; reg < 4; ++reg) {
          const int row = wm * 64 + i * 16 + g4 + 4 * reg;
          const int col = wn * 64 + j * 16 + r16;
          out[row * TBM + col] = acc[i][j][reg];
        }
  } else {
    const bool interior = (tm + 1) * TBM <= pr.M && (tn + 1) * TBM <= pr.N;
    const double exp_ca = exp_nonpos_ca();
    double sb[4];
#pragma unroll
    for (int j = 0; j < 4; ++j) {
      const int col = tn * TBM + wn * 64 + j * 16 + r16;
      sb[j] = (EPI != 3 && col < pr.N) ? P.sqb[col] : 0.0;
    }
#pragma unroll
    for (int i = 0; i < 4; ++i)
#pragma unroll
      for (int reg = 0; reg < 4; ++reg) {
        const int row = tm * TBM + wm * 64 + i * 16 + g4 + 4 * reg;
        if (!interior && row >= pr.M) continue;
        const double sa = EPI != 3 ? P.sqa[row] : 0.0;
        double* orow = P.out + (int64_t)row * P.ldo + tn * TBM + wn * 64 + r16;
#pragma unroll
        for (int j = 0; j < 4; ++j) {
          const double dot = acc[i][j][reg];
          double v;
          if (EPI == 3) {
            v = dot + P.sigma0sq;
          } else {
            const double D = fmax(sa + sb[j] - 2.0 * dot, 0.0);
            if (EPI == 1) {
              v = exp_nonpos(-0.5 * D, exp_ca);
            } else if (EPI == 4) {
              v = tps_value(D);
            } else {
              const double t = sqrt(D) * 2.23606797749978969641;
              v = (1.0 + t + t * t / 3.0) * exp_nonpos(-t, exp_ca);
            }
          }
          if (interior || tn * TBM + wn * 64 + j * 16 + r16 < pr.N) orow[j * 16] = v;
        }
      }
  }
}

template <int EPI>
__global__ void __launch_bounds__(256, 2) gemm_tn_f64_kernel(TnParams P) {
  tn_body<EPI>(P);
}
__global__ void __launch_bounds__(256, 2) gram_fused_f64_kernel(TnParams P) {
  tn_body<0>(P);
}
template <int EPI>
__global__ void __launch_bounds__(256, 2) gemm_tn_f64_kernel_batched(const nk::ArgPack<TnParams>* table) {
  tn_body<EPI>(table[blockIdx.z].v);
}
__global__ void __launch_bounds__(256, 2) gram_fused_f64_kernel_batched(const nk::ArgPack<TnParams>* table) {
  tn_body<0>(table[blockIdx.z].v);
}
#define NK_TN_TWIN(E)                                                                                                   \
  static nk::TwinReg tn_twin_reg_##E(reinterpret_cast<const void*>(static_cast<void (*)(TnParams)>(gemm_tn_f64_kernel<E>)), \
                                     reinterpret_cast<const void*>(gemm_tn_f64_kernel_batched<E>),                        \
                                     sizeof(nk::ArgPack<TnParams>), "gemm_tn_f64_kernel<" #E ">");
NK_TN_TWIN(0) NK_TN_TWIN(1) NK_TN_TWIN(2) NK_TN_TWIN(3) NK_TN_TWIN(4)
static nk::TwinReg gram_fused_twin_reg(reinterpret_cast<const void*>(static_cast<void (*)(TnParams)>(gram_fused_f64_kernel)),
                                       reinterpret_cast<const void*>(gram_fused_f64_kernel_batched),
                                       sizeof(nk::ArgPack<TnParams>), "gram_fused_f64_kernel");

__device__ __forceinline__ void gemm_tn_reduce_kernel_body(const TnRedParams& P) {
  __shared__ double sh[16][130];
  if (P.skip_state != nullptr) {
    const double f = P.skip_state[0];
    if (f != 0.0 && f <= (double)P.skip_step) return;
  }
  const int gt = blockIdx.x / RPARTS, part = blockIdx.x % RPARTS;
  int pi = 0;
#pragma unroll
  for (int q = 1; q < TN_MAXP; ++q)
    if (q < P.nprob && gt >= P.p[q].tile_begin) pi = q;
  const TnRed pr = P.p[pi];
  int tm, tn;
  tn_tile_coords(gt - pr.tile_begin, pr.tri, pr.tiles_n, pr.M, tm, tn);
  typedef double d2 __attribute__((ext_vector_type(2)));
  const double* base = P.slab + (int64_t)gt * P.splitk * (TBM * TBM) + part * (16 * TBM) + threadIdx.x * 2;
  d2 s[4];
#pragma unroll
  for (int i = 0; i < 4; ++i) s[i] = d2{0.0, 0.0};
  for (int k = 0; k < P.splitk; ++k) {
    const double* bk = base + (int64_t)k * (TBM * TBM);
#pragma unroll
    for (int i = 0; i < 4; ++i) s[i] += *reinterpret_cast<const d2*>(bk + 512 * i);
  }
  const bool mirror = pr.tri == TRI_UPPER_MIRROR && tm != tn;
  const bool transposed = mirror || pr.Ct != nullptr;
  const int row0 = tm * TBM + part * 16, col0 = tn * TBM;
  double rsum = 0.0;
#pragma unroll
  for (int i = 0; i < 4; ++i) {
    const int idx = threadIdx.x * 2 + 512 * i;
    const int r = idx >> 7, c = idx & 127;
    const int row = row0 + r;
#pragma unroll
    for (int h = 0; h < 2; ++h) {
      const int col = col0 + c + h;
      double v = 0.0;
      if (row < pr.M && col < pr.N) {
        v = pr.alpha * s[i][h];
        if (pr.beta != 0.0) v += pr.beta * pr.C[(int64_t)row * pr.ldc + col];
        pr.C[(int64_t)row * pr.ldc + col] = v;
        if (pr.Caff) pr.Caff[(int64_t)row * pr.ldc + col] = pr.aff_a * v + (row == col ? pr.aff_c : 0.0);
        const double e = v - (row == col ? 1.0 : 0.0);
        rsum = fma(e, e, rsum);
      }
      if (transposed) sh[r][c + h] = v;
    }
  }
  if (P.resid_partials != nullptr) {
    __shared__ double wsum[4];
#pragma unroll
    for (int off = 32; off > 0; off >>= 1) rsum += __shfl_down(rsum, off, 64);
    if ((threadIdx.x & 63) == 0) wsum[threadIdx.x >> 6] = rsum;
    __syncthreads();
    if (threadIdx.x == 0) {
      const double w = (wsum[0] + wsum[1]) + (wsum[2] + wsum[3]);
      P.resid_partials[blockIdx.x] = mirror ? 2.0 * w : w;
    }
  }
  if (!transposed) return;
  __syncthreads();
  const int c = threadIdx.x >> 1, rb = (threadIdx.x & 1) * 8;
  const int col = col0 + c;
  if (col >= pr.N) return;
#pragma unroll
  for (int q = 0; q < 8; ++q) {
    const int row = row0 + rb + q;
    if (row >= pr.M) break;
    const double v = sh[rb + q][c];
    if (mirror) pr.C[(int64_t)col * pr.ldc + row] = v;
    if (pr.Ct) pr.Ct[(int64_t)col * pr.ldct + row] = v;
    if (mirror && pr.Caff) pr.Caff[(int64_t)col * pr.ldc + row] = pr.aff_a * v;
  }
}
__global__ void __launch_bounds__(256) gemm_tn_reduce_kernel(TnRedParams P) { gemm_tn_reduce_kernel_body(P); }
__global__ void __launch_bounds__(256) gemm_tn_reduce_kernel_batched(const nk::ArgPack<TnRedParams>* table) {
  gemm_tn_reduce_kernel_body(table[blockIdx.z].v);
}
static nk::TwinReg gemm_tn_reduce_twin_reg(reinterpret_cast<const void*>(static_cast<void (*)(TnRedParams)>(gemm_tn_reduce_kernel)),
                                           reinterpret_cast<const void*>(gemm_tn_reduce_kernel_batched),
                                           sizeof(nk::ArgPack<TnRedParams>), "gemm_tn_reduce_kernel");

int launch_tn_reduce(nk_ctx* ctx, const TnRedParams& R, int ntiles) {
  hipLaunchKernelGGL(gemm_tn_reduce_kernel, dim3((unsigned)ntiles * RPARTS), dim3(256), 0, ctx->stream, R);
  NK_HIP(hipGetLastError());
  return NK_OK;
}

__device__ __forceinline__ void transpose_kernel_body(const double* __restrict__ src, int64_t lds_, double* __restrict__ dst, int64_t ldd, int rows, int cols) {
  __shared__ double tile[32][33];
  const int bx = blockIdx.x * 32, by = blockIdx.y * 32;
  const int tx = threadIdx.x & 31, ty = threadIdx.x >> 5;
  for (int r = ty; r < 32; r += 8) {
    const int row = by + r, col = bx + tx;
    if (row < rows && col < cols) tile[r][tx] = src[(int64_t)row * lds_ + col];
  }
  __syncthreads();
  for (int r = ty; r < 32; r += 8) {
    const int orow = bx + r, ocol = by + tx;
    if (orow < cols && ocol < rows) dst[(int64_t)orow * ldd + ocol] = tile[tx][r];
  }
}
__global__ void __launch_bounds__(256) transpose_kernel(const double* __restrict__ src, int64_t lds_, double* __restrict__ dst, int64_t ldd, int rows, int cols) { transpose_kernel_body(src, lds_, dst, ldd, rows, cols); }
NK_BATCHED_TWIN(transpose_kernel, (256), const double*, int64_t, double*, int64_t, int, int)

int launch_transpose(nk_ctx* ctx, const double* src, int64_t lds_, double* dst, int64_t ldd, int rows, int cols) {
  if (rows <= 0 || cols <= 0) return NK_OK;
  dim3 grid((cols + 31) / 32, (rows + 31) / 32);
  hipLaunchKernelGGL(transpose_kernel, grid, dim3(256), 0, ctx->stream, src, lds_, dst, ldd, rows, cols);
  NK_HIP(hipGetLastError());
  return NK_OK;
}

static inline bool aligned16(const void* p) { return (reinterpret_cast<uintptr_t>(p) & 15) == 0; }

bool tn_fast_ok(const TnProblem& p) {
  return p.M >= 2 && p.N >= 2 && aligned16(p.A) && aligned16(p.B) && p.lda % 2 == 0 && p.ldb % 2 == 0 &&
         p.lda >= ((p.M + 1) & ~1) && p.ldb >= ((p.N + 1) & ~1);
}

static bool g_tn_attr_set = false;
static int tn_use_asm() {
  const char* e = getenv("NYSKOOP_TN_ASM");
  return (e && e[0] == '0') ? 0 : 1;
}

int tn_ensure_zero_page(nk_ctx* ctx) {
  if (ctx->d_zeros) return NK_OK;
  NK_HIP(hipMalloc(reinterpret_cast<void**>(&ctx->d_zeros), 4096));
  NK_HIP(hipMemset(ctx->d_zeros, 0, 4096));
  return NK_OK;
}

int launch_gemm_tn_multi(nk_ctx* ctx, const TnProblem* probs, int nprob, int64_t K, int splitk, float* ms_kernel,
                         bool sync_timing, const TnSkip* skip) {
  NK_REQUIRE(nprob >= 1 && nprob <= TN_MAXP, "gemm_tn_multi: 1..4 problems");
// ... 1 lines not shown
  NK_TRY(tn_ensure_zero_page(ctx));
  TnParams P;
  TnRedParams R;
  int ntiles = 0;
  for (int q = 0; q < nprob; ++q) {
    const TnProblem& s = probs[q];
    NK_REQUIRE(tn_fast_ok(s), "gemm_tn_multi: problem %d violates the alignment contract", q);
    NK_REQUIRE(s.tri == TRI_FULL || (s.tri == TRI_UPPER_MIRROR && s.M == s.N), "gemm_tn_multi: bad tri mode");
    const int tmn = (s.M + TBM - 1) / TBM, tnn = (s.N + TBM - 1) / TBM;
    TnDev& d = P.p[q];
    d.A = s.A; d.B = s.B; d.lda = s.lda; d.ldb = s.ldb; d.M = s.M; d.N = s.N;
    d.tiles_n = tnn; d.tri = s.tri; d.ktrim = s.ktrim; d.tile_begin = ntiles;
    d.C = s.C; d.ldc = s.ldc; d.alpha = s.alpha; d.beta = s.beta; d.Ct = s.Ct; d.ldct = s.ldct;
    d.A_even = s.A_even; d.B_even = s.B_even;
    d.Caff = s.Caff; d.aff_a = s.aff_a; d.aff_c = s.aff_c;
    TnRed& r = R.p[q];
    r.Caff = s.Caff; r.aff_a = s.aff_a; r.aff_c = s.aff_c;
    r.Ct = s.Ct; r.ldct = s.ldct;
    r.C = s.C; r.ldc = s.ldc; r.M = s.M; r.N = s.N; r.tiles_n = tnn; r.tri = s.tri; r.tile_begin = ntiles;
    r.alpha = s.alpha; r.beta = s.beta;
    ntiles += s.tri == TRI_FULL ? tmn * tnn : tmn * (tmn + 1) / 2;
  }
  for (int q = nprob; q < TN_MAXP; ++q) {
    P.p[q] = P.p[0];
    P.p[q].tile_begin = 1 << 30;
    R.p[q] = R.p[0];
    R.p[q].tile_begin = 1 << 30;
  }
  const int ktiles_total = (int)((K + TBK - 1) / TBK);
  const bool want_resid = skip && skip->resid_partials != nullptr;
  if (splitk <= 0) {
    const int slots = 2 * ctx->num_cu;
    const int max_split = ktiles_total / 8 > 1 ? ktiles_total / 8 : 1;
    double best = 1e300;
    splitk = 1;
    for (int c = 1; c <= 64 && c <= max_split; ++c) {
      const int64_t wgs = (int64_t)ntiles * c;
      const double steps = (double)((ktiles_total + c - 1) / c);
      const int64_t full = wgs / slots, rem = wgs % slots;
      double t = full * 2.44 * steps;
      if (rem > 0) t += (rem <= ctx->num_cu ? 2.35 : 2.44) * steps;
      t *= 4096.0;
      if (c > 1) t += (double)wgs * (TBM * TBM * 8.0 * 2.0) / 4.0e12 * 2.4e9;
      t += 2000.0 * c / 8.0;
      if (c % 8 == 0) t *= 0.97;
      if (t < best) { best = t; splitk = c; }
    }
  }
  if (want_resid && splitk < 2) splitk = 2;
  if (nprob >= 3 && getenv("NYSKOOP_TN_SPLITK")) splitk = atoi(getenv("NYSKOOP_TN_SPLITK"));
  P.kmask = getenv("NYSKOOP_TN_KMASK") ? (int)strtol(getenv("NYSKOOP_TN_KMASK"), nullptr, 0) : -1;
  P.use_asm = tn_use_asm();
  P.nprob = nprob; P.ntiles = ntiles; P.K = (int)K; P.splitk = splitk;
  P.klen = ((ktiles_total + splitk - 1) / splitk) * TBK;
  if (P.klen == 0) P.klen = TBK;
  P.zeros = ctx->d_zeros;
  const ArenaMark mark = arena_mark(ctx);
  double* slab = nullptr;
  if (splitk > 1) NK_TRY(arena_alloc_t(ctx, (size_t)ntiles * splitk * TBM * TBM, &slab));
  P.slab = slab;
  R.nprob = nprob; R.splitk = splitk; R.slab = slab;
  P.skip_state = R.skip_state = skip ? skip->state : nullptr;
  P.skip_step = R.skip_step = skip ? skip->step : 0;
  P.select_state = skip ? skip->select : nullptr;
  R.resid_partials = (skip && splitk > 1 && nprob == 1) ? skip->resid_partials : nullptr;
  if (skip && skip->resid_count) *skip->resid_count = R.resid_partials ? ntiles * RPARTS : 0;
  if (!g_tn_attr_set) {
    NK_HIP(hipFuncSetAttribute(reinterpret_cast<const void*>(gemm_tn_f64_kernel<0>),
                               hipFuncAttributeMaxDynamicSharedMemorySize, TN_LDS_BYTES));
    NK_HIP(hipFuncSetAttribute(reinterpret_cast<const void*>(gram_fused_f64_kernel),
                               hipFuncAttributeMaxDynamicSharedMemorySize, TN_LDS_BYTES));
    NK_HIP(hipFuncSetAttribute(reinterpret_cast<const void*>(gemm_tn_f64_kernel<1>),
                               hipFuncAttributeMaxDynamicSharedMemorySize, TN_LDS_BYTES));
    NK_HIP(hipFuncSetAttribute(reinterpret_cast<const void*>(gemm_tn_f64_kernel<2>),
                               hipFuncAttributeMaxDynamicSharedMemorySize, TN_LDS_BYTES));
    NK_HIP(hipFuncSetAttribute(reinterpret_cast<const void*>(gemm_tn_f64_kernel<3>),
                               hipFuncAttributeMaxDynamicSharedMemorySize, TN_LDS_BYTES));
    NK_HIP(hipFuncSetAttribute(reinterpret_cast<const void*>(gemm_tn_f64_kernel<4>),
                               hipFuncAttributeMaxDynamicSharedMemorySize, TN_LDS_BYTES));
    NK_HIP(hipFuncSetAttribute(reinterpret_cast<const void*>(gemm_tn_f64_kernel_batched<0>),
                               hipFuncAttributeMaxDynamicSharedMemorySize, TN_LDS_BYTES));
    NK_HIP(hipFuncSetAttribute(reinterpret_cast<const void*>(gemm_tn_f64_kernel_batched<1>),
                               hipFuncAttributeMaxDynamicSharedMemorySize, TN_LDS_BYTES));
    NK_HIP(hipFuncSetAttribute(reinterpret_cast<const void*>(gemm_tn_f64_kernel_batched<2>),
                               hipFuncAttributeMaxDynamicSharedMemorySize, TN_LDS_BYTES));
    NK_HIP(hipFuncSetAttribute(reinterpret_cast<const void*>(gemm_tn_f64_kernel_batched<3>),
                               hipFuncAttributeMaxDynamicSharedMemorySize, TN_LDS_BYTES));
    NK_HIP(hipFuncSetAttribute(reinterpret_cast<const void*>(gemm_tn_f64_kernel_batched<4>),
                               hipFuncAttributeMaxDynamicSharedMemorySize, TN_LDS_BYTES));
    NK_HIP(hipFuncSetAttribute(reinterpret_cast<const void*>(gram_fused_f64_kernel_batched),
                               hipFuncAttributeMaxDynamicSharedMemorySize, TN_LDS_BYTES));
    g_tn_attr_set = true;
  }
  if (ms_kernel) NK_HIP(hipEventRecord(ctx->ev[14], ctx->stream));
  P.sqa = P.sqb = nullptr; P.out = nullptr; P.ldo = 0; P.ktype = 0; P.sigma0sq = 0.0;
  if (nprob >= 3)
    hipLaunchKernelGGL(gram_fused_f64_kernel, dim3((unsigned)(ntiles * splitk)), dim3(256), TN_LDS_BYTES, ctx->stream, P);
  else
    hipLaunchKernelGGL(gemm_tn_f64_kernel<0>, dim3((unsigned)(ntiles * splitk)), dim3(256), TN_LDS_BYTES, ctx->stream, P);
  NK_HIP(hipGetLastError());
  if (ms_kernel) NK_HIP(hipEventRecord(ctx->ev[15], ctx->stream));
  if (splitk > 1) {
    hipLaunchKernelGGL(gemm_tn_reduce_kernel, dim3((unsigned)ntiles * RPARTS), dim3(256), 0, ctx->stream, R);
    NK_HIP(hipGetLastError());
  }
  if (ms_kernel && sync_timing) {
    NK_HIP(hipEventSynchronize(ctx->ev[15]));
    NK_HIP(hipEventElapsedTime(ms_kernel, ctx->ev[14], ctx->ev[15]));
  }
  arena_release(ctx, mark);
  return NK_OK;
}


__device__ __forceinline__ void prep_rows_kernel_body(const double* __restrict__ X, int64_t ldx, int rows, int d, const double* __restrict__ winv, const double* __restrict__ center, double* __restrict__ Xt, int64_t ldt) {
  __shared__ double tile[32][33];
  const int k0 = blockIdx.x * 32, r0 = blockIdx.y * 32;
  const int tx = threadIdx.x & 31, ty = threadIdx.x >> 5;
  for (int r = ty; r < 32; r += 8) {
    const int row = r0 + r, k = k0 + tx;
    if (row < rows && k < d) tile[r][tx] = (X[(int64_t)row * ldx + k] - center[k]) * winv[k];
  }
  __syncthreads();
  for (int r = ty; r < 32; r += 8) {
    const int k = k0 + r, row = r0 + tx;
    if (k < d && row < rows) Xt[(int64_t)k * ldt + row] = tile[tx][r];
  }
}
__global__ void __launch_bounds__(256) prep_rows_kernel(const double* __restrict__ X, int64_t ldx, int rows, int d, const double* __restrict__ winv, const double* __restrict__ center, double* __restrict__ Xt, int64_t ldt) { prep_rows_kernel_body(X, ldx, rows, d, winv, center, Xt, ldt); }
NK_BATCHED_TWIN(prep_rows_kernel, (256), const double*, int64_t, int, int, const double*, const double*, double*, int64_t)
__device__ __forceinline__ void colsq_kernel_body(const double* __restrict__ Xt, int64_t ldt, int rows, int d, double* __restrict__ sq) {
  __shared__ double part[4][64];
  const int lane = threadIdx.x & 63, w = threadIdx.x >> 6;
  const int i = blockIdx.x * 64 + lane;
  double s0 = 0.0, s1 = 0.0, s2 = 0.0, s3 = 0.0;
  if (i < rows) {
    int k = w;
    for (; k + 12 < d; k += 16) {
      const double v0 = Xt[(int64_t)k * ldt + i], v1 = Xt[(int64_t)(k + 4) * ldt + i];
      const double v2 = Xt[(int64_t)(k + 8) * ldt + i], v3 = Xt[(int64_t)(k + 12) * ldt + i];
      s0 = fma(v0, v0, s0); s1 = fma(v1, v1, s1); s2 = fma(v2, v2, s2); s3 = fma(v3, v3, s3);
    }
    for (; k < d; k += 4) {
      const double v = Xt[(int64_t)k * ldt + i];
      s0 = fma(v, v, s0);
    }
  }
  part[w][lane] = (s0 + s1) + (s2 + s3);
  __syncthreads();
  if (w == 0 && i < rows) sq[i] = (part[0][lane] + part[1][lane]) + (part[2][lane] + part[3][lane]);
}
__global__ void __launch_bounds__(256) colsq_kernel(const double* __restrict__ Xt, int64_t ldt, int rows, int d, double* __restrict__ sq) { colsq_kernel_body(Xt, ldt, rows, d, sq); }
NK_BATCHED_TWIN(colsq_kernel, (256), const double*, int64_t, int, int, double*)
__device__ __forceinline__ void colsum_partial_kernel_body(const double* __restrict__ Z, int64_t ldz, int rows, int d, int rows_per_chunk, double* __restrict__ partial) {
  const int k = blockIdx.x * blockDim.x + threadIdx.x;
  if (k >= d) return;
  const int r0 = blockIdx.y * rows_per_chunk;
  const int r1 = min(rows, r0 + rows_per_chunk);
  double s = 0.0;
  for (int r = r0; r < r1; ++r) s += Z[(int64_t)r * ldz + k];
  partial[(int64_t)blockIdx.y * d + k] = s;
}
__global__ void __launch_bounds__(256) colsum_partial_kernel(const double* __restrict__ Z, int64_t ldz, int rows, int d, int rows_per_chunk, double* __restrict__ partial) { colsum_partial_kernel_body(Z, ldz, rows, d, rows_per_chunk, partial); }
NK_BATCHED_TWIN(colsum_partial_kernel, (256), const double*, int64_t, int, int, int, double*)
__device__ __forceinline__ void colmean_finish_kernel_body(const double* __restrict__ partial, int chunks, int rows, int d, double* __restrict__ mean) {
  const int k = blockIdx.x * blockDim.x + threadIdx.x;
  if (k >= d) return;
  double s = 0.0;
  for (int c = 0; c < chunks; ++c) s += partial[(int64_t)c * d + k];
  mean[k] = s / rows;
}
__global__ void __launch_bounds__(256) colmean_finish_kernel(const double* __restrict__ partial, int chunks, int rows, int d, double* __restrict__ mean) { colmean_finish_kernel_body(partial, chunks, rows, d, mean); }
NK_BATCHED_TWIN(colmean_finish_kernel, (256), const double*, int, int, int, double*)

int launch_colmean(nk_ctx* ctx, const double* Z, int64_t ldz, int rows, int d, double* mean) {
  const ArenaMark mk = arena_mark(ctx);
  const int rpc = 32;
  const int chunks = (rows + rpc - 1) / rpc;
  double* partial = nullptr;
  NK_TRY(arena_alloc_t(ctx, (size_t)chunks * d, &partial));
  hipLaunchKernelGGL(colsum_partial_kernel, dim3((d + 255) / 256, chunks), dim3(256), 0, ctx->stream, Z, ldz, rows, d, rpc,
                     partial);
  hipLaunchKernelGGL(colmean_finish_kernel, dim3((d + 255) / 256), dim3(256), 0, ctx->stream, partial, chunks, rows, d, mean);
  NK_HIP(hipGetLastError());
  arena_release(ctx, mk);
  return NK_OK;
}

int prep_rows(nk_ctx* ctx, const double* X, int64_t ldx, int64_t rows, int d, const double* winv, const double* center,
              double* Xt, int64_t ldt, double* sq) {
  dim3 grid((d + 31) / 32, (unsigned)((rows + 31) / 32));
  hipLaunchKernelGGL(prep_rows_kernel, grid, dim3(256), 0, ctx->stream, X, ldx, (int)rows, d, winv, center, Xt, ldt);
  hipLaunchKernelGGL(colsq_kernel, dim3((unsigned)((rows + 63) / 64)), dim3(256), 0, ctx->stream, Xt, ldt, (int)rows, d, sq);
  NK_HIP(hipGetLastError());
  return NK_OK;
}

int launch_kmat_gram(nk_ctx* ctx, int ktype, const double* At, int64_t ldat, const double* sqa, int64_t nA,
                     const double* Bt, int64_t ldbt, const double* sqb, int64_t nB, int d, double sigma0, double* out,
                     int64_t ldo) {
  NK_TRY(tn_ensure_zero_page(ctx));
  TnProblem tp;
  tp.A = At; tp.B = Bt; tp.lda = ldat; tp.ldb = ldbt; tp.M = (int)nA; tp.N = (int)nB;
  NK_REQUIRE(tn_fast_ok(tp), "kmat_gram: operands violate the alignment contract");
  TnParams P;
  P.skip_state = nullptr; P.skip_step = 0; P.select_state = nullptr;
  const int tmn = (int)((nA + TBM - 1) / TBM), tnn = (int)((nB + TBM - 1) / TBM);
  TnDev& dv = P.p[0];
  dv.A = At; dv.B = Bt; dv.lda = ldat; dv.ldb = ldbt; dv.M = (int)nA; dv.N = (int)nB; dv.tiles_n = tnn; dv.tri = TRI_FULL;
  dv.tile_begin = 0; dv.ktrim = KTRIM_NONE; dv.A_even = dv.B_even = nullptr; dv.Caff = nullptr; dv.aff_a = dv.aff_c = 0.0;
  dv.C = nullptr; dv.ldc = 0; dv.alpha = 1.0; dv.beta = 0.0; dv.Ct = nullptr; dv.ldct = 0;
  for (int q = 1; q < TN_MAXP; ++q) { P.p[q] = P.p[0]; P.p[q].tile_begin = 1 << 30; }
  P.nprob = 1; P.ntiles = tmn * tnn; P.K = d; P.splitk = 1; P.kmask = -1; P.use_asm = tn_use_asm();
  P.klen = ((d + TBK - 1) / TBK) * TBK;
  P.zeros = ctx->d_zeros; P.slab = nullptr;
  P.sqa = sqa; P.sqb = sqb; P.out = out; P.ldo = ldo; P.ktype = ktype; P.sigma0sq = sigma0 * sigma0;
  if (!g_tn_attr_set) {
    NK_HIP(hipFuncSetAttribute(reinterpret_cast<const void*>(gemm_tn_f64_kernel<0>),
                               hipFuncAttributeMaxDynamicSharedMemorySize, TN_LDS_BYTES));
    NK_HIP(hipFuncSetAttribute(reinterpret_cast<const void*>(gram_fused_f64_kernel),
                               hipFuncAttributeMaxDynamicSharedMemorySize, TN_LDS_BYTES));
    NK_HIP(hipFuncSetAttribute(reinterpret_cast<const void*>(gemm_tn_f64_kernel<1>),
                               hipFuncAttributeMaxDynamicSharedMemorySize, TN_LDS_BYTES));
    NK_HIP(hipFuncSetAttribute(reinterpret_cast<const void*>(gemm_tn_f64_kernel<2>),
                               hipFuncAttributeMaxDynamicSharedMemorySize, TN_LDS_BYTES));
    NK_HIP(hipFuncSetAttribute(reinterpret_cast<const void*>(gemm_tn_f64_kernel<3>),
                               hipFuncAttributeMaxDynamicSharedMemorySize, TN_LDS_BYTES));
    NK_HIP(hipFuncSetAttribute(reinterpret_cast<const void*>(gemm_tn_f64_kernel<4>),
                               hipFuncAttributeMaxDynamicSharedMemorySize, TN_LDS_BYTES));
    NK_HIP(hipFuncSetAttribute(reinterpret_cast<const void*>(gemm_tn_f64_kernel_batched<0>),
                               hipFuncAttributeMaxDynamicSharedMemorySize, TN_LDS_BYTES));
    NK_HIP(hipFuncSetAttribute(reinterpret_cast<const void*>(gemm_tn_f64_kernel_batched<1>),
                               hipFuncAttributeMaxDynamicSharedMemorySize, TN_LDS_BYTES));
    NK_HIP(hipFuncSetAttribute(reinterpret_cast<const void*>(gemm_tn_f64_kernel_batched<2>),
                               hipFuncAttributeMaxDynamicSharedMemorySize, TN_LDS_BYTES));
    NK_HIP(hipFuncSetAttribute(reinterpret_cast<const void*>(gemm_tn_f64_kernel_batched<3>),
                               hipFuncAttributeMaxDynamicSharedMemorySize, TN_LDS_BYTES));
    NK_HIP(hipFuncSetAttribute(reinterpret_cast<const void*>(gemm_tn_f64_kernel_batched<4>),
                               hipFuncAttributeMaxDynamicSharedMemorySize, TN_LDS_BYTES));
    NK_HIP(hipFuncSetAttribute(reinterpret_cast<const void*>(gram_fused_f64_kernel_batched),
                               hipFuncAttributeMaxDynamicSharedMemorySize, TN_LDS_BYTES));
    g_tn_attr_set = true;
  }
  const unsigned grid = 8u * (unsigned)tmn * (unsigned)((tnn + 7) / 8);
  if (ktype == NK_KERNEL_RBF)
    hipLaunchKernelGGL(gemm_tn_f64_kernel<1>, dim3(grid), dim3(256), TN_LDS_BYTES, ctx->stream, P);
  else if (ktype == NK_KERNEL_MATERN52)
    hipLaunchKernelGGL(gemm_tn_f64_kernel<2>, dim3(grid), dim3(256), TN_LDS_BYTES, ctx->stream, P);
  else if (ktype == NK_KERNEL_TPS)
    hipLaunchKernelGGL(gemm_tn_f64_kernel<4>, dim3(grid), dim3(256), TN_LDS_BYTES, ctx->stream, P);
  else
    hipLaunchKernelGGL(gemm_tn_f64_kernel<3>, dim3(grid), dim3(256), TN_LDS_BYTES, ctx->stream, P);
  NK_HIP(hipGetLastError());
  return NK_OK;
}

}
```

### nys_koop_lqr_amd/csrc/nk_tn_kstep.inc

```
#define NK_TN_KSTEPS_ASM \
  "s_mov_b64 s[92:93], %[rowa]\n\t" \
  "s_mov_b64 s[94:95], %[rowb]\n\t" \
  "s_cmp_eq_u32 %[cnt], 0\n\t" \
  "s_cbranch_scc1 nk_tn_after_%=\n\t" \
  "nk_tn_loop_%=:\n\t" \
  "s_waitcnt lgkmcnt(0)\n\t" \
  "v_mfma_f64_16x16x4_f64 %[c00], %[a00], %[b00], %[c00]\n\t" \
  "ds_read_b64 %[a10], %[ard0] offset:4608\n\t" \
  "v_mfma_f64_16x16x4_f64 %[c01], %[a00], %[b01], %[c01]\n\t" \
  "ds_read_b64 %[a11], %[ard0] offset:4736\n\t" \
  "v_mfma_f64_16x16x4_f64 %[c02], %[a00], %[b02], %[c02]\n\t" \
  "ds_read_b64 %[a12], %[ard0] offset:4864\n\t" \
  "v_mfma_f64_16x16x4_f64 %[c03], %[a00], %[b03], %[c03]\n\t" \
  "ds_read_b64 %[a13], %[ard0] offset:4992\n\t" \
  "v_mfma_f64_16x16x4_f64 %[c10], %[a01], %[b00], %[c10]\n\t" \
  "ds_read_b64 %[b10], %[brd0] offset:4608\n\t" \
  "v_mfma_f64_16x16x4_f64 %[c11], %[a01], %[b01], %[c11]\n\t" \
  "ds_read_b64 %[b11], %[brd0] offset:4736\n\t" \
  "v_mfma_f64_16x16x4_f64 %[c12], %[a01], %[b02], %[c12]\n\t" \
  "ds_read_b64 %[b12], %[brd0] offset:4864\n\t" \
  "v_mfma_f64_16x16x4_f64 %[c13], %[a01], %[b03], %[c13]\n\t" \
  "ds_read_b64 %[b13], %[brd0] offset:4992\n\t" \
  "v_mfma_f64_16x16x4_f64 %[c20], %[a02], %[b00], %[c20]\n\t" \
  "s_mov_b32 m0, %[dst1]\n\t" \
// ... 440 lines not shown
  "ds_read_b64 %[b01], %[brd1] offset:9344\n\t" \
  "v_mfma_f64_16x16x4_f64 %[c12], %[a11], %[b12], %[c12]\n\t" \
  "ds_read_b64 %[b02], %[brd1] offset:9472\n\t" \
  "v_mfma_f64_16x16x4_f64 %[c13], %[a11], %[b13], %[c13]\n\t" \
  "ds_read_b64 %[b03], %[brd1] offset:9600\n\t" \
  "v_mfma_f64_16x16x4_f64 %[c20], %[a12], %[b10], %[c20]\n\t" \
  "v_mfma_f64_16x16x4_f64 %[c21], %[a12], %[b11], %[c21]\n\t" \
  "v_mfma_f64_16x16x4_f64 %[c22], %[a12], %[b12], %[c22]\n\t" \
  "v_mfma_f64_16x16x4_f64 %[c23], %[a12], %[b13], %[c23]\n\t" \
  "v_mfma_f64_16x16x4_f64 %[c30], %[a13], %[b10], %[c30]\n\t" \
  "v_mfma_f64_16x16x4_f64 %[c31], %[a13], %[b11], %[c31]\n\t" \
  "v_mfma_f64_16x16x4_f64 %[c32], %[a13], %[b12], %[c32]\n\t" \
  "v_mfma_f64_16x16x4_f64 %[c33], %[a13], %[b13], %[c33]\n\t" \
  "s_waitcnt lgkmcnt(0)\n\t" \
  "v_mfma_f64_16x16x4_f64 %[c00], %[a00], %[b00], %[c00]\n\t" \
  "ds_read_b64 %[a10], %[ard1] offset:13824\n\t" \
  "v_mfma_f64_16x16x4_f64 %[c01], %[a00], %[b01], %[c01]\n\t" \
  "ds_read_b64 %[a11], %[ard1] offset:13952\n\t" \
  "v_mfma_f64_16x16x4_f64 %[c02], %[a00], %[b02], %[c02]\n\t" \
  "ds_read_b64 %[a12], %[ard1] offset:14080\n\t" \
  "v_mfma_f64_16x16x4_f64 %[c03], %[a00], %[b03], %[c03]\n\t" \
  "ds_read_b64 %[a13], %[ard1] offset:14208\n\t" \
  "v_mfma_f64_16x16x4_f64 %[c10], %[a01], %[b00], %[c10]\n\t" \
  "ds_read_b64 %[b10], %[brd1] offset:13824\n\t" \
  "v_mfma_f64_16x16x4_f64 %[c11], %[a01], %[b01], %[c11]\n\t" \
  "ds_read_b64 %[b11], %[brd1] offset:13952\n\t" \
  "v_mfma_f64_16x16x4_f64 %[c12], %[a01], %[b02], %[c12]\n\t" \
  "ds_read_b64 %[b12], %[brd1] offset:14080\n\t" \
  "v_mfma_f64_16x16x4_f64 %[c13], %[a01], %[b03], %[c13]\n\t" \
  "ds_read_b64 %[b13], %[brd1] offset:14208\n\t" \
  "v_mfma_f64_16x16x4_f64 %[c20], %[a02], %[b00], %[c20]\n\t" \
  "v_mfma_f64_16x16x4_f64 %[c21], %[a02], %[b01], %[c21]\n\t" \
  "v_mfma_f64_16x16x4_f64 %[c22], %[a02], %[b02], %[c22]\n\t" \
  "v_mfma_f64_16x16x4_f64 %[c23], %[a02], %[b03], %[c23]\n\t" \
  "v_mfma_f64_16x16x4_f64 %[c30], %[a03], %[b00], %[c30]\n\t" \
  "v_mfma_f64_16x16x4_f64 %[c31], %[a03], %[b01], %[c31]\n\t" \
  "v_mfma_f64_16x16x4_f64 %[c32], %[a03], %[b02], %[c32]\n\t" \
  "v_mfma_f64_16x16x4_f64 %[c33], %[a03], %[b03], %[c33]\n\t" \
  "s_waitcnt lgkmcnt(0)\n\t" \
  "v_mfma_f64_16x16x4_f64 %[c00], %[a10], %[b10], %[c00]\n\t" \
  "v_mfma_f64_16x16x4_f64 %[c01], %[a10], %[b11], %[c01]\n\t" \
  "v_mfma_f64_16x16x4_f64 %[c02], %[a10], %[b12], %[c02]\n\t" \
  "v_mfma_f64_16x16x4_f64 %[c03], %[a10], %[b13], %[c03]\n\t" \
  "v_mfma_f64_16x16x4_f64 %[c10], %[a11], %[b10], %[c10]\n\t" \
  "v_mfma_f64_16x16x4_f64 %[c11], %[a11], %[b11], %[c11]\n\t" \
  "v_mfma_f64_16x16x4_f64 %[c12], %[a11], %[b12], %[c12]\n\t" \
  "v_mfma_f64_16x16x4_f64 %[c13], %[a11], %[b13], %[c13]\n\t" \
  "v_mfma_f64_16x16x4_f64 %[c20], %[a12], %[b10], %[c20]\n\t" \
  "v_mfma_f64_16x16x4_f64 %[c21], %[a12], %[b11], %[c21]\n\t" \
  "v_mfma_f64_16x16x4_f64 %[c22], %[a12], %[b12], %[c22]\n\t" \
  "v_mfma_f64_16x16x4_f64 %[c23], %[a12], %[b13], %[c23]\n\t" \
  "v_mfma_f64_16x16x4_f64 %[c30], %[a13], %[b10], %[c30]\n\t" \
  "v_mfma_f64_16x16x4_f64 %[c31], %[a13], %[b11], %[c31]\n\t" \
  "v_mfma_f64_16x16x4_f64 %[c32], %[a13], %[b12], %[c32]\n\t" \
  "v_mfma_f64_16x16x4_f64 %[c33], %[a13], %[b13], %[c33]\n\t" \
  "s_branch nk_tn_end_%=\n\t" \
  "nk_tn_even_%=:\n\t" \
  "s_bitcmp1_b32 %[flags], 1\n\t" \
  "s_cbranch_scc0 nk_tn_end_%=\n\t" \
  "s_waitcnt lgkmcnt(0)\n\t" \
  "v_mfma_f64_16x16x4_f64 %[c00], %[a00], %[b00], %[c00]\n\t" \
  "ds_read_b64 %[a10], %[ard0] offset:4608\n\t" \
  "v_mfma_f64_16x16x4_f64 %[c01], %[a00], %[b01], %[c01]\n\t" \
  "ds_read_b64 %[a11], %[ard0] offset:4736\n\t" \
  "v_mfma_f64_16x16x4_f64 %[c02], %[a00], %[b02], %[c02]\n\t" \
  "ds_read_b64 %[a12], %[ard0] offset:4864\n\t" \
  "v_mfma_f64_16x16x4_f64 %[c03], %[a00], %[b03], %[c03]\n\t" \
  "ds_read_b64 %[a13], %[ard0] offset:4992\n\t" \
  "v_mfma_f64_16x16x4_f64 %[c10], %[a01], %[b00], %[c10]\n\t" \
  "ds_read_b64 %[b10], %[brd0] offset:4608\n\t" \
  "v_mfma_f64_16x16x4_f64 %[c11], %[a01], %[b01], %[c11]\n\t" \
  "ds_read_b64 %[b11], %[brd0] offset:4736\n\t" \
  "v_mfma_f64_16x16x4_f64 %[c12], %[a01], %[b02], %[c12]\n\t" \
  "ds_read_b64 %[b12], %[brd0] offset:4864\n\t" \
  "v_mfma_f64_16x16x4_f64 %[c13], %[a01], %[b03], %[c13]\n\t" \
  "ds_read_b64 %[b13], %[brd0] offset:4992\n\t" \
  "v_mfma_f64_16x16x4_f64 %[c20], %[a02], %[b00], %[c20]\n\t" \
  "v_mfma_f64_16x16x4_f64 %[c21], %[a02], %[b01], %[c21]\n\t" \
  "v_mfma_f64_16x16x4_f64 %[c22], %[a02], %[b02], %[c22]\n\t" \
  "v_mfma_f64_16x16x4_f64 %[c23], %[a02], %[b03], %[c23]\n\t" \
  "v_mfma_f64_16x16x4_f64 %[c30], %[a03], %[b00], %[c30]\n\t" \
  "v_mfma_f64_16x16x4_f64 %[c31], %[a03], %[b01], %[c31]\n\t" \
  "v_mfma_f64_16x16x4_f64 %[c32], %[a03], %[b02], %[c32]\n\t" \
  "v_mfma_f64_16x16x4_f64 %[c33], %[a03], %[b03], %[c33]\n\t" \
  "s_waitcnt lgkmcnt(0)\n\t" \
  "v_mfma_f64_16x16x4_f64 %[c00], %[a10], %[b10], %[c00]\n\t" \
  "ds_read_b64 %[a00], %[ard0] offset:9216\n\t" \
  "v_mfma_f64_16x16x4_f64 %[c01], %[a10], %[b11], %[c01]\n\t" \
  "ds_read_b64 %[a01], %[ard0] offset:9344\n\t" \
  "v_mfma_f64_16x16x4_f64 %[c02], %[a10], %[b12], %[c02]\n\t" \
  "ds_read_b64 %[a02], %[ard0] offset:9472\n\t" \
  "v_mfma_f64_16x16x4_f64 %[c03], %[a10], %[b13], %[c03]\n\t" \
  "ds_read_b64 %[a03], %[ard0] offset:9600\n\t" \
  "v_mfma_f64_16x16x4_f64 %[c10], %[a11], %[b10], %[c10]\n\t" \
  "ds_read_b64 %[b00], %[brd0] offset:9216\n\t" \
  "v_mfma_f64_16x16x4_f64 %[c11], %[a11], %[b11], %[c11]\n\t" \
  "ds_read_b64 %[b01], %[brd0] offset:9344\n\t" \
  "v_mfma_f64_16x16x4_f64 %[c12], %[a11], %[b12], %[c12]\n\t" \
  "ds_read_b64 %[b02], %[brd0] offset:9472\n\t" \
  "v_mfma_f64_16x16x4_f64 %[c13], %[a11], %[b13], %[c13]\n\t" \
  "ds_read_b64 %[b03], %[brd0] offset:9600\n\t" \
  "v_mfma_f64_16x16x4_f64 %[c20], %[a12], %[b10], %[c20]\n\t" \
  "v_mfma_f64_16x16x4_f64 %[c21], %[a12], %[b11], %[c21]\n\t" \
  "v_mfma_f64_16x16x4_f64 %[c22], %[a12], %[b12], %[c22]\n\t" \
  "v_mfma_f64_16x16x4_f64 %[c23], %[a12], %[b13], %[c23]\n\t" \
  "v_mfma_f64_16x16x4_f64 %[c30], %[a13], %[b10], %[c30]\n\t" \
  "v_mfma_f64_16x16x4_f64 %[c31], %[a13], %[b11], %[c31]\n\t" \
  "v_mfma_f64_16x16x4_f64 %[c32], %[a13], %[b12], %[c32]\n\t" \
  "v_mfma_f64_16x16x4_f64 %[c33], %[a13], %[b13], %[c33]\n\t" \
  "s_waitcnt lgkmcnt(0)\n\t" \
  "v_mfma_f64_16x16x4_f64 %[c00], %[a00], %[b00], %[c00]\n\t" \
  "ds_read_b64 %[a10], %[ard0] offset:13824\n\t" \
  "v_mfma_f64_16x16x4_f64 %[c01], %[a00], %[b01], %[c01]\n\t" \
  "ds_read_b64 %[a11], %[ard0] offset:13952\n\t" \
  "v_mfma_f64_16x16x4_f64 %[c02], %[a00], %[b02], %[c02]\n\t" \
  "ds_read_b64 %[a12], %[ard0] offset:14080\n\t" \
  "v_mfma_f64_16x16x4_f64 %[c03], %[a00], %[b03], %[c03]\n\t" \
  "ds_read_b64 %[a13], %[ard0] offset:14208\n\t" \
  "v_mfma_f64_16x16x4_f64 %[c10], %[a01], %[b00], %[c10]\n\t" \
  "ds_read_b64 %[b10], %[brd0] offset:13824\n\t" \
  "v_mfma_f64_16x16x4_f64 %[c11], %[a01], %[b01], %[c11]\n\t" \
  "ds_read_b64 %[b11], %[brd0] offset:13952\n\t" \
  "v_mfma_f64_16x16x4_f64 %[c12], %[a01], %[b02], %[c12]\n\t" \
  "ds_read_b64 %[b12], %[brd0] offset:14080\n\t" \
  "v_mfma_f64_16x16x4_f64 %[c13], %[a01], %[b03], %[c13]\n\t" \
  "ds_read_b64 %[b13], %[brd0] offset:14208\n\t" \
  "v_mfma_f64_16x16x4_f64 %[c20], %[a02], %[b00], %[c20]\n\t" \
  "v_mfma_f64_16x16x4_f64 %[c21], %[a02], %[b01], %[c21]\n\t" \
  "v_mfma_f64_16x16x4_f64 %[c22], %[a02], %[b02], %[c22]\n\t" \
  "v_mfma_f64_16x16x4_f64 %[c23], %[a02], %[b03], %[c23]\n\t" \
  "v_mfma_f64_16x16x4_f64 %[c30], %[a03], %[b00], %[c30]\n\t" \
  "v_mfma_f64_16x16x4_f64 %[c31], %[a03], %[b01], %[c31]\n\t" \
  "v_mfma_f64_16x16x4_f64 %[c32], %[a03], %[b02], %[c32]\n\t" \
  "v_mfma_f64_16x16x4_f64 %[c33], %[a03], %[b03], %[c33]\n\t" \
  "s_waitcnt lgkmcnt(0)\n\t" \
  "v_mfma_f64_16x16x4_f64 %[c00], %[a10], %[b10], %[c00]\n\t" \
  "v_mfma_f64_16x16x4_f64 %[c01], %[a10], %[b11], %[c01]\n\t" \
  "v_mfma_f64_16x16x4_f64 %[c02], %[a10], %[b12], %[c02]\n\t" \
  "v_mfma_f64_16x16x4_f64 %[c03], %[a10], %[b13], %[c03]\n\t" \
  "v_mfma_f64_16x16x4_f64 %[c10], %[a11], %[b10], %[c10]\n\t" \
  "v_mfma_f64_16x16x4_f64 %[c11], %[a11], %[b11], %[c11]\n\t" \
  "v_mfma_f64_16x16x4_f64 %[c12], %[a11], %[b12], %[c12]\n\t" \
  "v_mfma_f64_16x16x4_f64 %[c13], %[a11], %[b13], %[c13]\n\t" \
  "v_mfma_f64_16x16x4_f64 %[c20], %[a12], %[b10], %[c20]\n\t" \
  "v_mfma_f64_16x16x4_f64 %[c21], %[a12], %[b11], %[c21]\n\t" \
  "v_mfma_f64_16x16x4_f64 %[c22], %[a12], %[b12], %[c22]\n\t" \
  "v_mfma_f64_16x16x4_f64 %[c23], %[a12], %[b13], %[c23]\n\t" \
  "v_mfma_f64_16x16x4_f64 %[c30], %[a13], %[b10], %[c30]\n\t" \
  "v_mfma_f64_16x16x4_f64 %[c31], %[a13], %[b11], %[c31]\n\t" \
  "v_mfma_f64_16x16x4_f64 %[c32], %[a13], %[b12], %[c32]\n\t" \
  "v_mfma_f64_16x16x4_f64 %[c33], %[a13], %[b13], %[c33]\n\t" \
  "nk_tn_end_%=:\n\t" \
  ""
```

Baseline: 24.54.

## Add BK=8 kernel-matrix GEMM variant and fused row-prep/square-norm kernel

Adds a K-tile-8 variant of the TN f64 MFMA kernel-matrix GEMM with its own hand-scheduled asm k-step loop. It uses half the LDS and a launch bound of 3 blocks per CU, aiming for higher occupancy on the K_nm build, and is enabled by default when d is divisible by 8. It also fuses the row centering/scaling transpose with the squared-norm computation into one persistent kernel, removing a second pass over Xt. A new nk_kernel_block_gram API and event counters are added. The risk is that the shorter K tile gives more barriers per FLOP and less latency hiding.

```diff
diff --git a/include/nyskoop.h b/include/nyskoop.h
--- a/include/nyskoop.h
+++ b/include/nyskoop.h
@@ -106,6 +106,9 @@
                      const double* B, int64_t ldb, int64_t nB,
                      double* out, int64_t ldo);
 
+int nk_kernel_block_gram(nk_ctx* ctx, const nk_kernel_desc* kd, const double* X, int64_t ldx, int64_t n, const double* Z,
+                         int64_t ldz, int64_t m, double* out, int64_t ldo, double* Xt, int64_t ldxt, double* sq);
+
 int nk_nystrom_fit(nk_ctx* ctx, const nk_kernel_desc* kd,
                    const double* X, int64_t ldx, const double* Y, int64_t ldy,
                    int64_t n, int32_t d, int32_t p,
diff --git a/nys_koop_lqr_amd/_lib.py b/nys_koop_lqr_amd/_lib.py
--- a/nys_koop_lqr_amd/_lib.py
+++ b/nys_koop_lqr_amd/_lib.py
@@ -81,6 +81,7 @@
     "nk_host_alloc": (_P, [C.c_uint64]),
     "nk_host_free": (None, [_P]),
     "nk_kernel_matrix": (C.c_int, [_P, C.POINTER(KernelDesc), _P, _I64, _I64, _P, _I64, _I64, _P, _I64]),
+    "nk_kernel_block_gram": (C.c_int, [_P, C.POINTER(KernelDesc), _P, _I64, _I64, _P, _I64, _I64, _P, _I64, _P, _I64, _P]),
     "nk_nystrom_fit": (C.c_int, [_P, C.POINTER(KernelDesc), _P, _I64, _P, _I64, _I64, _I32, _I32,
                                  C.POINTER(_I64), _I32, _P, _I64, _P, _I64, _I32, _D, _D,
                                  C.POINTER(_P), C.POINTER(FitStats)]),
diff --git a/nys_koop_lqr_amd/csrc/nk_api.hip b/nys_koop_lqr_amd/csrc/nk_api.hip
--- a/nys_koop_lqr_amd/csrc/nk_api.hip
+++ b/nys_koop_lqr_amd/csrc/nk_api.hip
@@ -373,6 +373,9 @@
     return NK_ERR_NO_DEVICE;
   }
   NK_REQUIRE(device >= 0 && device < n, "nk_create: device %d out of range (0..%d)", device, n - 1);
+  const char* kmat_bk_env = getenv("NYSKOOP_KMAT_BK");
+  NK_REQUIRE(!kmat_bk_env || strcmp(kmat_bk_env, "8") == 0 || strcmp(kmat_bk_env, "16") == 0,
+             "nk_create: NYSKOOP_KMAT_BK must be 8 or 16");
   NK_HIP(hipSetDevice(device));
   hipDeviceProp_t prop;
   NK_HIP(hipGetDeviceProperties(&prop, device));
@@ -410,6 +413,8 @@
   for (int i = 0; i < 8; ++i) NK_HIP(hipEventCreateWithFlags(&ctx->ev_up[i], hipEventDisableTiming));
   const char* km = getenv("NYSKOOP_KMAT");
   ctx->kmat_mode = (km && strcmp(km, "direct") == 0) ? 1 : 0;
+  if (kmat_bk_env) ctx->kmat_bk = atoi(kmat_bk_env);
+  if (const char* pf = getenv("NYSKOOP_PREP_FUSED")) ctx->prep_fused = atoi(pf) != 0 ? 1 : 0;
   const char* st = getenv("NYSKOOP_STRICT_SPD");
   ctx->strict_spd = (st && atoi(st) != 0) ? 1 : 0;
   if (const char* rp = getenv("NYSKOOP_REFINE_PIVOT")) ctx->refine_pivot = atof(rp);
@@ -841,6 +846,49 @@
   return NK_OK;
 }
 
+int nk_kernel_block_gram(nk_ctx* ctx, const nk_kernel_desc* kd, const double* X, int64_t ldx, int64_t n, const double* Z,
+                         int64_t ldz, int64_t m, double* out, int64_t ldo, double* Xt, int64_t ldxt, double* sq) {
+  NK_TRY(check_ctx(ctx));
+  NK_REQUIRE(kd && X && Z && out, "nk_kernel_block_gram: null argument");
+  NK_REQUIRE(n >= 2 && m >= 2 && n < (1LL << 31) && m < (1LL << 31) && kd->d > 0, "nk_kernel_block_gram: bad size");
+  NK_REQUIRE(ldx >= kd->d && ldz >= kd->d && ldo >= m && (Xt == nullptr || ldxt >= n),
+             "nk_kernel_block_gram: leading dimension too small");
+  const int d = kd->d;
+  double* winv = nullptr;
+  NK_TRY(arena_alloc_t(ctx, (size_t)d, &winv));
+  NK_TRY(make_winv(ctx, kd, d, winv));
+  MatIn x, z;
+  NK_TRY(stage_in(ctx, X, ldx, n, d, &x));
+  NK_TRY(stage_in(ctx, Z, ldz, m, d, &z));
+  MatOut o, oxt, osq;
+  NK_TRY(stage_out(ctx, out, ldo, n, m, &o));
+  const int64_t ltx = (n + 1) & ~(int64_t)1, ltz = (m + 1) & ~(int64_t)1;
+  double *center = nullptr, *Rt = nullptr, *sqr = nullptr, *Zt = nullptr, *sqz = nullptr;
+  NK_TRY(arena_alloc_t(ctx, (size_t)d, &center));
+  NK_TRY(arena_alloc_t(ctx, (size_t)d * ltx, &Rt));
+  NK_TRY(arena_alloc_t(ctx, (size_t)n, &sqr));
+  NK_TRY(arena_alloc_t(ctx, (size_t)d * ltz, &Zt));
+  NK_TRY(arena_alloc_t(ctx, (size_t)m, &sqz));
+  if (kd->type == NK_KERNEL_LINEAR) NK_TRY(launch_fill(ctx, center, d, 1, d, 0.0));
+  else NK_TRY(launch_colmean(ctx, z.ptr, z.ld, (int)m, d, center));
+  NK_TRY(prep_rows(ctx, z.ptr, z.ld, m, d, winv, center, Zt, ltz, sqz));
+  NK_TRY(prep_rows(ctx, x.ptr, x.ld, n, d, winv, center, Rt, ltx, sqr));
+  NK_TRY(launch_kmat_gram(ctx, kd->type, Rt, ltx, sqr, n, Zt, ltz, sqz, m, d, kd->sigma0, o.dev, o.ld));
+  NK_TRY(finish_out(ctx, o));
+  if (Xt) {
+    NK_TRY(stage_out(ctx, Xt, ldxt, d, n, &oxt));
+    NK_TRY(launch_copy2d(ctx, Rt, ltx, oxt.dev, oxt.ld, d, n));
+    NK_TRY(finish_out(ctx, oxt));
+  }
+  if (sq) {
+    NK_TRY(stage_out(ctx, sq, n, 1, n, &osq));
+    NK_TRY(launch_copy2d(ctx, sqr, n, osq.dev, osq.ld, 1, n));
+    NK_TRY(finish_out(ctx, osq));
+  }
+  NK_HIP(hipStreamSynchronize(ctx->stream));
+  return NK_OK;
+}
+
 static inline size_t gram_block1(int m, int p) { return (((size_t)(2 * m + p) * (m + p)) + 1) & ~(size_t)1; }
 static inline size_t gram_doubles(int m, int d, int p) { return gram_block1(m, p) + (size_t)(m + d) * m; }
 
diff --git a/nys_koop_lqr_amd/csrc/nk_common.h b/nys_koop_lqr_amd/csrc/nk_common.h
--- a/nys_koop_lqr_amd/csrc/nk_common.h
+++ b/nys_koop_lqr_amd/csrc/nk_common.h
@@ -76,6 +76,8 @@
   hipEvent_t ev[16];
   int num_cu = 256;
   int kmat_mode = 0;
+  int kmat_bk = 8;
+  int prep_fused = 1;
   double refine_pivot = 0.0;
   int refine_steps = 2;
   int strict_spd = 0;
@@ -212,7 +214,7 @@
 int group_leave(nk_ctx* c);
 void group_stats(nk_ctx* c, uint64_t out[4]);
 enum { CNT_CHAIN_GIVEUP = 0, CNT_JACOBI_GIVEUP = 1, CNT_RANK_TRUNCATED = 2, CNT_SQRT_RETRY = 3, CNT_REFINED = 4,
-       CNT_CHOL_FLOW_GIVEUP = 5, CNT_CHOL_FLOW = 6, CNT_N = 7 };
+       CNT_CHOL_FLOW_GIVEUP = 5, CNT_CHOL_FLOW = 6, CNT_KMAT_BK8 = 7, CNT_KMAT_BK16 = 8, CNT_PREP_FUSED = 9, CNT_N = 10 };
 void count_event(int which);
 uint64_t read_counter(int which);
 hipError_t real_stream_sync(hipStream_t s);
diff --git a/nys_koop_lqr_amd/csrc/nk_gemm_tn.hip b/nys_koop_lqr_amd/csrc/nk_gemm_tn.hip
--- a/nys_koop_lqr_amd/csrc/nk_gemm_tn.hip
+++ b/nys_koop_lqr_amd/csrc/nk_gemm_tn.hip
@@ -13,6 +13,8 @@
 constexpr int TSTRIDE = 144;
 constexpr int TSTAGE = 2 * TBK * TSTRIDE;
 constexpr int TN_LDS_BYTES = 2 * TSTAGE * 8;
+constexpr int TBK8 = 8;
+constexpr int TN8_LDS_BYTES = 2 * (2 * TBK8 * TSTRIDE) * 8;
 
 struct TnDev {
   const double* A;
@@ -66,8 +68,10 @@
 }
 __device__ __forceinline__ void dma_wait_all() { asm volatile("s_waitcnt vmcnt(0)" ::: "memory"); }
 
-template <int EPI>
+template <int EPI, int BK = TBK>
 __device__ __forceinline__ void tn_body(const TnParams& P) {
+  constexpr int TBK = BK;
+  constexpr int TSTAGE = 2 * BK * TSTRIDE;
   extern __shared__ __attribute__((aligned(16))) double smem[];
   const int split = blockIdx.x % P.splitk;
   const int gt = blockIdx.x / P.splitk;
@@ -116,14 +120,14 @@
     const int k0 = kbeg + kt * TBK;
     if (k0 + TBK <= kend) {
 #pragma unroll
-      for (int q = 0; q < 4; ++q) {
+      for (int q = 0; q < BK / 4; ++q) {
         const int r = wave + 4 * q;
         dma_row(opA + (int64_t)((k0 + r) & P.kmask) * pr.lda, offa, sa + (uint32_t)(r * TSTRIDE) * 8u);
         dma_row(opB + (int64_t)((k0 + r) & P.kmask) * pr.ldb, offb, sb + (uint32_t)(r * TSTRIDE) * 8u);
       }
     } else {
 #pragma unroll
-      for (int q = 0; q < 4; ++q) {
+      for (int q = 0; q < BK / 4; ++q) {
         const int r = wave + 4 * q;
         const int k = k0 + r;
         if (k < kend) {
@@ -184,13 +188,15 @@
 #define NK_TN_IN_OPERANDS                                                                                             \
   [ard0] "v"(ard0), [brd0] "v"(brd0), [ard1] "v"(ard1), [brd1] "v"(brd1), [voa] "v"(offa), [vob] "v"(offb),           \
       [rowa] "s"(rowa), [rowb] "s"(rowb), [stra] "s"(stra), [strb] "s"(strb), [dst0] "s"(dst0), [dst1] "s"(dst1)
+#define NK_TN8_IN_OPERANDS                                                                                            \
+  [ard0] "v"(ard0), [brd0] "v"(brd0), [voa] "v"(offa), [vob] "v"(offb), [rowa] "s"(rowa), [rowb] "s"(rowb),           \
+      [stra] "s"(stra), [strb] "s"(strb), [dst0] "s"(dst0), [dst1] "s"(dst1)
 #define NK_TN_CLOBBERS "memory", "m0", "scc", "s92", "s93", "s94", "s95"
   const int nfull = (kend - kbeg) / TBK;
   int kt_start = 0;
   if (P.kmask == -1 && P.use_asm && nfull >= 1) {
     const uint32_t dst0 = (uint32_t)__builtin_amdgcn_readfirstlane(lds0 + (uint32_t)(wave * TSTRIDE) * 8u);
     const uint32_t dst1 = dst0 + STAGE_B;
-    const uint32_t ard1 = ard0 + STAGE_B, brd1 = brd0 + STAGE_B;
     const int steady = nfull - 1;
     uint32_t cnt = (uint32_t)__builtin_amdgcn_readfirstlane((uint32_t)(steady / 2));
     const uint32_t flags =
@@ -198,11 +204,20 @@
     kt_start = 2 * (int)cnt + (int)(flags & 1) + (int)(flags >> 1);
     const uint64_t rowa = uniform_u64((uint64_t)(uintptr_t)(opA + (int64_t)(kbeg + TBK + wave) * pr.lda));
     const uint64_t rowb = uniform_u64((uint64_t)(uintptr_t)(opB + (int64_t)(kbeg + TBK + wave) * pr.ldb));
-    if (kt_start > 0)
-      asm volatile(NK_TN_KSTEPS_ASM
-                   : NK_TN_ACC_OPERANDS, [cnt] "+s"(cnt)
-                   : NK_TN_IN_OPERANDS, [flags] "s"(flags)
-                   : NK_TN_CLOBBERS);
+    if constexpr (BK == 16) {
+      const uint32_t ard1 = ard0 + STAGE_B, brd1 = brd0 + STAGE_B;
+      if (kt_start > 0)
+        asm volatile(NK_TN_KSTEPS_ASM
+                     : NK_TN_ACC_OPERANDS, [cnt] "+s"(cnt)
+                     : NK_TN_IN_OPERANDS, [flags] "s"(flags)
+                     : NK_TN_CLOBBERS);
+    } else {
+      if (kt_start > 0)
+        asm volatile(NK_TN8_KSTEPS_ASM
+                     : NK_TN_ACC_OPERANDS, [cnt] "+s"(cnt)
+                     : NK_TN8_IN_OPERANDS, [flags] "s"(flags)
+                     : NK_TN_CLOBBERS);
+    }
   }
   for (int kt = kt_start; kt < ktiles; ++kt) {
     const int st = kt & 1;
@@ -211,14 +226,16 @@
     if (more) issue(kt + 1, st ^ 1);
     mma(a0, b0);
     __builtin_amdgcn_sched_barrier(0);
-    frag(st, 2, a0, b0);
-    __builtin_amdgcn_sched_barrier(0);
-    mma(a1, b1);
-    __builtin_amdgcn_sched_barrier(0);
-    frag(st, 3, a1, b1);
-    __builtin_amdgcn_sched_barrier(0);
-    mma(a0, b0);
-    __builtin_amdgcn_sched_barrier(0);
+    if constexpr (BK == 16) {
+      frag(st, 2, a0, b0);
+      __builtin_amdgcn_sched_barrier(0);
+      mma(a1, b1);
+      __builtin_amdgcn_sched_barrier(0);
+      frag(st, 3, a1, b1);
+      __builtin_amdgcn_sched_barrier(0);
+      mma(a0, b0);
+      __builtin_amdgcn_sched_barrier(0);
+    }
     dma_wait_all();
     __syncthreads();
     if (more) frag(st ^ 1, 0, a0, b0);
@@ -307,6 +324,11 @@
 }
 __global__ void __launch_bounds__(256, 2) gram_fused_f64_kernel(TnParams P) {
   tn_body<0>(P);
+}
+template <int EPI>
+__global__ void __launch_bounds__(256, 3) kmat_bk8_f64_kernel(TnParams P) {
+  static_assert(EPI >= 1, "kernel-matrix epilogues only");
+  tn_body<EPI, TBK8>(P);
 }
 template <int EPI>
 __global__ void __launch_bounds__(256, 2) gemm_tn_f64_kernel_batched(const nk::ArgPack<TnParams>* table) {
@@ -614,6 +636,53 @@
 }
 __global__ void __launch_bounds__(256) colsq_kernel(const double* __restrict__ Xt, int64_t ldt, int rows, int d, double* __restrict__ sq) { colsq_kernel_body(Xt, ldt, rows, d, sq); }
 NK_BATCHED_TWIN(colsq_kernel, (256), const double*, int64_t, int, int, double*)
+__global__ void __launch_bounds__(256, 4) prep_rows_sq_kernel(const double* __restrict__ X, int64_t ldx, int rows, int d, const double* __restrict__ winv, const double* __restrict__ center, double* __restrict__ Xt, int64_t ldt, double* __restrict__ sq, int nblocks) {
+  __shared__ double tile[64][33];
+  __shared__ double part[4][64];
+  const int tx = threadIdx.x & 31, ty = threadIdx.x >> 5;
+  const int lane = threadIdx.x & 63, w = threadIdx.x >> 6;
+  const int nchunk = (d + 31) / 32;
+  const int tmain = d > w + 12 ? 4 * ((d - w - 12 + 15) / 16) : 0;
+  for (int blk = blockIdx.x; blk < nblocks; blk += gridDim.x) {
+    const int r0 = blk * 64;
+    const int i = r0 + lane;
+    double v[8];
+    auto load = [&](int c) {
+      const int k = c * 32 + tx;
+      const double ce = k < d ? center[k] : 0.0, wi = k < d ? winv[k] : 0.0;
+#pragma unroll
+      for (int q = 0; q < 8; ++q) {
+        const int row = r0 + ty + 8 * q;
+        v[q] = (row < rows && k < d) ? (X[(int64_t)row * ldx + k] - ce) * wi : 0.0;
+      }
+    };
+    double s0 = 0.0, s1 = 0.0, s2 = 0.0, s3 = 0.0;
+    load(0);
+    for (int c = 0; c < nchunk; ++c) {
+      __syncthreads();
+#pragma unroll
+      for (int q = 0; q < 8; ++q) tile[ty + 8 * q][tx] = v[q];
+      __syncthreads();
+      if (c + 1 < nchunk) load(c + 1);
+#pragma unroll
+      for (int j = 0; j < 8; ++j) {
+        const int k = c * 32 + w + 4 * j;
+        if (k < d) {
+          const double x = tile[lane][w + 4 * j];
+          if (i < rows) Xt[(int64_t)k * ldt + i] = x;
+          const bool rest = c * 8 + j >= tmain;
+          if (rest || (j & 3) == 0) s0 = fma(x, x, s0);
+          else if ((j & 3) == 1) s1 = fma(x, x, s1);
+          else if ((j & 3) == 2) s2 = fma(x, x, s2);
+          else s3 = fma(x, x, s3);
+        }
+      }
+    }
+    part[w][lane] = (s0 + s1) + (s2 + s3);
+    __syncthreads();
+    if (w == 0 && i < rows) sq[i] = (part[0][lane] + part[1][lane]) + (part[2][lane] + part[3][lane]);
+  }
+}
 __device__ __forceinline__ void colsum_partial_kernel_body(const double* __restrict__ Z, int64_t ldz, int rows, int d, int rows_per_chunk, double* __restrict__ partial) {
   const int k = blockIdx.x * blockDim.x + threadIdx.x;
   if (k >= d) return;
@@ -651,6 +720,15 @@
 
 int prep_rows(nk_ctx* ctx, const double* X, int64_t ldx, int64_t rows, int d, const double* winv, const double* center,
               double* Xt, int64_t ldt, double* sq) {
+  const int64_t nblocks = (rows + 63) / 64;
+  if (ctx->prep_fused && nblocks >= ctx->num_cu && !ctx_recording(ctx)) {
+    const int64_t per = (nblocks + 4 * (int64_t)ctx->num_cu - 1) / (4 * (int64_t)ctx->num_cu);
+    hipLaunchKernelGGL(prep_rows_sq_kernel, dim3((unsigned)((nblocks + per - 1) / per)), dim3(256), 0, ctx->stream, X, ldx,
+                       (int)rows, d, winv, center, Xt, ldt, sq, (int)nblocks);
+    NK_HIP(hipGetLastError());
+    count_event(CNT_PREP_FUSED);
+    return NK_OK;
+  }
   dim3 grid((d + 31) / 32, (unsigned)((rows + 31) / 32));
   hipLaunchKernelGGL(prep_rows_kernel, grid, dim3(256), 0, ctx->stream, X, ldx, (int)rows, d, winv, center, Xt, ldt);
   hipLaunchKernelGGL(colsq_kernel, dim3((unsigned)((rows + 63) / 64)), dim3(256), 0, ctx->stream, Xt, ldt, (int)rows, d, sq);
@@ -705,6 +783,20 @@
     g_tn_attr_set = true;
   }
   const unsigned grid = 8u * (unsigned)tmn * (unsigned)((tnn + 7) / 8);
+  if (ctx->kmat_bk == 8 && d % TBK8 == 0 && !ctx_recording(ctx)) {
+    if (ktype == NK_KERNEL_RBF)
+      hipLaunchKernelGGL(kmat_bk8_f64_kernel<1>, dim3(grid), dim3(256), TN8_LDS_BYTES, ctx->stream, P);
+    else if (ktype == NK_KERNEL_MATERN52)
+      hipLaunchKernelGGL(kmat_bk8_f64_kernel<2>, dim3(grid), dim3(256), TN8_LDS_BYTES, ctx->stream, P);
+    else if (ktype == NK_KERNEL_TPS)
+      hipLaunchKernelGGL(kmat_bk8_f64_kernel<4>, dim3(grid), dim3(256), TN8_LDS_BYTES, ctx->stream, P);
+    else
+      hipLaunchKernelGGL(kmat_bk8_f64_kernel<3>, dim3(grid), dim3(256), TN8_LDS_BYTES, ctx->stream, P);
+    NK_HIP(hipGetLastError());
+    count_event(CNT_KMAT_BK8);
+    return NK_OK;
+  }
+  count_event(CNT_KMAT_BK16);
   if (ktype == NK_KERNEL_RBF)
     hipLaunchKernelGGL(gemm_tn_f64_kernel<1>, dim3(grid), dim3(256), TN_LDS_BYTES, ctx->stream, P);
   else if (ktype == NK_KERNEL_MATERN52)
diff --git a/nys_koop_lqr_amd/csrc/nk_tn_kstep.inc b/nys_koop_lqr_amd/csrc/nk_tn_kstep.inc
--- a/nys_koop_lqr_amd/csrc/nk_tn_kstep.inc
+++ b/nys_koop_lqr_amd/csrc/nk_tn_kstep.inc
@@ -616,3 +616,317 @@
   "v_mfma_f64_16x16x4_f64 %[c33], %[a13], %[b13], %[c33]\n\t" \
   "nk_tn_end_%=:\n\t" \
   ""
+#define NK_TN8_KSTEPS_ASM \
+  "s_mov_b64 s[92:93], %[rowa]\n\t" \
+  "s_mov_b64 s[94:95], %[rowb]\n\t" \
+  "s_cmp_eq_u32 %[cnt], 0\n\t" \
+  "s_cbranch_scc1 nk_tn8_after_%=\n\t" \
+  "nk_tn8_loop_%=:\n\t" \
+  "s_waitcnt lgkmcnt(0)\n\t" \
+  "v_mfma_f64_16x16x4_f64 %[c00], %[a00], %[b00], %[c00]\n\t" \
+  "ds_read_b64 %[a10], %[ard0] offset:4608\n\t" \
+  "s_mov_b32 m0, %[dst1]\n\t" \
+  "s_nop 0\n\t" \
+  "global_load_lds_dwordx4 %[voa], s[92:93]\n\t" \
+  "v_mfma_f64_16x16x4_f64 %[c01], %[a00], %[b01], %[c01]\n\t" \
+  "ds_read_b64 %[a11], %[ard0] offset:4736\n\t" \
+  "s_add_u32 m0, m0, 9216\n\t" \
+  "s_add_u32 s92, s92, %[stra]\n\t" \
+  "s_addc_u32 s93, s93, 0\n\t" \
+  "v_mfma_f64_16x16x4_f64 %[c02], %[a00], %[b02], %[c02]\n\t" \
+  "ds_read_b64 %[a12], %[ard0] offset:4864\n\t" \
+  "global_load_lds_dwordx4 %[vob], s[94:95]\n\t" \
+  "s_sub_u32 m0, m0, 4608\n\t" \
+  "s_add_u32 s94, s94, %[strb]\n\t" \
+  "v_mfma_f64_16x16x4_f64 %[c03], %[a00], %[b03], %[c03]\n\t" \
+  "ds_read_b64 %[a13], %[ard0] offset:4992\n\t" \
+  "s_addc_u32 s95, s95, 0\n\t" \
+  "s_nop 0\n\t" \
+  "global_load_lds_dwordx4 %[voa], s[92:93]\n\t" \
+  "v_mfma_f64_16x16x4_f64 %[c10], %[a01], %[b00], %[c10]\n\t" \
+  "ds_read_b64 %[b10], %[brd0] offset:4608\n\t" \
+  "s_add_u32 m0, m0, 9216\n\t" \
+  "s_add_u32 s92, s92, %[stra]\n\t" \
+  "s_addc_u32 s93, s93, 0\n\t" \
+  "v_mfma_f64_16x16x4_f64 %[c11], %[a01], %[b01], %[c11]\n\t" \
+  "ds_read_b64 %[b11], %[brd0] offset:4736\n\t" \
+  "global_load_lds_dwordx4 %[vob], s[94:95]\n\t" \
+  "s_add_u32 s94, s94, %[strb]\n\t" \
+  "s_addc_u32 s95, s95, 0\n\t" \
+  "v_mfma_f64_16x16x4_f64 %[c12], %[a01], %[b02], %[c12]\n\t" \
+  "ds_read_b64 %[b12], %[brd0] offset:4864\n\t" \
+  "v_mfma_f64_16x16x4_f64 %[c13], %[a01], %[b03], %[c13]\n\t" \
+  "ds_read_b64 %[b13], %[brd0] offset:4992\n\t" \
+  "v_mfma_f64_16x16x4_f64 %[c20], %[a02], %[b00], %[c20]\n\t" \
+  "v_mfma_f64_16x16x4_f64 %[c21], %[a02], %[b01], %[c21]\n\t" \
+  "v_mfma_f64_16x16x4_f64 %[c22], %[a02], %[b02], %[c22]\n\t" \
+  "v_mfma_f64_16x16x4_f64 %[c23], %[a02], %[b03], %[c23]\n\t" \
+  "v_mfma_f64_16x16x4_f64 %[c30], %[a03], %[b00], %[c30]\n\t" \
+  "v_mfma_f64_16x16x4_f64 %[c31], %[a03], %[b01], %[c31]\n\t" \
+  "v_mfma_f64_16x16x4_f64 %[c32], %[a03], %[b02], %[c32]\n\t" \
+  "v_mfma_f64_16x16x4_f64 %[c33], %[a03], %[b03], %[c33]\n\t" \
+  "s_waitcnt lgkmcnt(0)\n\t" \
+  "v_mfma_f64_16x16x4_f64 %[c00], %[a10], %[b10], %[c00]\n\t" \
+  "v_mfma_f64_16x16x4_f64 %[c01], %[a10], %[b11], %[c01]\n\t" \
+  "v_mfma_f64_16x16x4_f64 %[c02], %[a10], %[b12], %[c02]\n\t" \
+  "v_mfma_f64_16x16x4_f64 %[c03], %[a10], %[b13], %[c03]\n\t" \
+  "v_mfma_f64_16x16x4_f64 %[c10], %[a11], %[b10], %[c10]\n\t" \
+  "v_mfma_f64_16x16x4_f64 %[c11], %[a11], %[b11], %[c11]\n\t" \
+  "v_mfma_f64_16x16x4_f64 %[c12], %[a11], %[b12], %[c12]\n\t" \
+  "v_mfma_f64_16x16x4_f64 %[c13], %[a11], %[b13], %[c13]\n\t" \
+  "s_waitcnt vmcnt(0)\n\t" \
+  "s_barrier\n\t" \
+  "v_mfma_f64_16x16x4_f64 %[c20], %[a12], %[b10], %[c20]\n\t" \
+  "ds_read_b64 %[a00], %[ard0] offset:18432\n\t" \
+  "ds_read_b64 %[a01], %[ard0] offset:18560\n\t" \
+  "v_mfma_f64_16x16x4_f64 %[c21], %[a12], %[b11], %[c21]\n\t" \
+  "ds_read_b64 %[a02], %[ard0] offset:18688\n\t" \
+  "ds_read_b64 %[a03], %[ard0] offset:18816\n\t" \
+  "v_mfma_f64_16x16x4_f64 %[c22], %[a12], %[b12], %[c22]\n\t" \
+  "ds_read_b64 %[b00], %[brd0] offset:18432\n\t" \
+  "ds_read_b64 %[b01], %[brd0] offset:18560\n\t" \
+  "v_mfma_f64_16x16x4_f64 %[c23], %[a12], %[b13], %[c23]\n\t" \
+  "ds_read_b64 %[b02], %[brd0] offset:18688\n\t" \
+  "ds_read_b64 %[b03], %[brd0] offset:18816\n\t" \
+  "v_mfma_f64_16x16x4_f64 %[c30], %[a13], %[b10], %[c30]\n\t" \
+  "v_mfma_f64_16x16x4_f64 %[c31], %[a13], %[b11], %[c31]\n\t" \
+  "v_mfma_f64_16x16x4_f64 %[c32], %[a13], %[b12], %[c32]\n\t" \
+  "v_mfma_f64_16x16x4_f64 %[c33], %[a13], %[b13], %[c33]\n\t" \
+  "s_waitcnt lgkmcnt(0)\n\t" \
+  "v_mfma_f64_16x16x4_f64 %[c00], %[a00], %[b00], %[c00]\n\t" \
+  "ds_read_b64 %[a10], %[ard0] offset:23040\n\t" \
+  "s_mov_b32 m0, %[dst0]\n\t" \
+  "s_nop 0\n\t" \
+  "global_load_lds_dwordx4 %[voa], s[92:93]\n\t" \
+  "v_mfma_f64_16x16x4_f64 %[c01], %[a00], %[b01], %[c01]\n\t" \
+  "ds_read_b64 %[a11], %[ard0] offset:23168\n\t" \
+  "s_add_u32 m0, m0, 9216\n\t" \
+  "s_add_u32 s92, s92, %[stra]\n\t" \
+  "s_addc_u32 s93, s93, 0\n\t" \
+  "v_mfma_f64_16x16x4_f64 %[c02], %[a00], %[b02], %[c02]\n\t" \
+  "ds_read_b64 %[a12], %[ard0] offset:23296\n\t" \
+  "global_load_lds_dwordx4 %[vob], s[94:95]\n\t" \
+  "s_sub_u32 m0, m0, 4608\n\t" \
+  "s_add_u32 s94, s94, %[strb]\n\t" \
+  "v_mfma_f64_16x16x4_f64 %[c03], %[a00], %[b03], %[c03]\n\t" \
+  "ds_read_b64 %[a13], %[ard0] offset:23424\n\t" \
+  "s_addc_u32 s95, s95, 0\n\t" \
+  "s_nop 0\n\t" \
+  "global_load_lds_dwordx4 %[voa], s[92:93]\n\t" \
+  "v_mfma_f64_16x16x4_f64 %[c10], %[a01], %[b00], %[c10]\n\t" \
+  "ds_read_b64 %[b10], %[brd0] offset:23040\n\t" \
+  "s_add_u32 m0, m0, 9216\n\t" \
+  "s_add_u32 s92, s92, %[stra]\n\t" \
+  "s_addc_u32 s93, s93, 0\n\t" \
+  "v_mfma_f64_16x16x4_f64 %[c11], %[a01], %[b01], %[c11]\n\t" \
+  "ds_read_b64 %[b11], %[brd0] offset:23168\n\t" \
+  "global_load_lds_dwordx4 %[vob], s[94:95]\n\t" \
+  "s_add_u32 s94, s94, %[strb]\n\t" \
+  "s_addc_u32 s95, s95, 0\n\t" \
+  "v_mfma_f64_16x16x4_f64 %[c12], %[a01], %[b02], %[c12]\n\t" \
+  "ds_read_b64 %[b12], %[brd0] offset:23296\n\t" \
+  "v_mfma_f64_16x16x4_f64 %[c13], %[a01], %[b03], %[c13]\n\t" \
+  "ds_read_b64 %[b13], %[brd0] offset:23424\n\t" \
+  "v_mfma_f64_16x16x4_f64 %[c20], %[a02], %[b00], %[c20]\n\t" \
+  "v_mfma_f64_16x16x4_f64 %[c21], %[a02], %[b01], %[c21]\n\t" \
+  "v_mfma_f64_16x16x4_f64 %[c22], %[a02], %[b02], %[c22]\n\t" \
+  "v_mfma_f64_16x16x4_f64 %[c23], %[a02], %[b03], %[c23]\n\t" \
+  "v_mfma_f64_16x16x4_f64 %[c30], %[a03], %[b00], %[c30]\n\t" \
+  "v_mfma_f64_16x16x4_f64 %[c31], %[a03], %[b01], %[c31]\n\t" \
+  "v_mfma_f64_16x16x4_f64 %[c32], %[a03], %[b02], %[c32]\n\t" \
+  "v_mfma_f64_16x16x4_f64 %[c33], %[a03], %[b03], %[c33]\n\t" \
+  "s_waitcnt lgkmcnt(0)\n\t" \
+  "v_mfma_f64_16x16x4_f64 %[c00], %[a10], %[b10], %[c00]\n\t" \
+  "v_mfma_f64_16x16x4_f64 %[c01], %[a10], %[b11], %[c01]\n\t" \
+  "v_mfma_f64_16x16x4_f64 %[c02], %[a10], %[b12], %[c02]\n\t" \
+  "v_mfma_f64_16x16x4_f64 %[c03], %[a10], %[b13], %[c03]\n\t" \
+  "v_mfma_f64_16x16x4_f64 %[c10], %[a11], %[b10], %[c10]\n\t" \
+  "v_mfma_f64_16x16x4_f64 %[c11], %[a11], %[b11], %[c11]\n\t" \
+  "v_mfma_f64_16x16x4_f64 %[c12], %[a11], %[b12], %[c12]\n\t" \
+  "v_mfma_f64_16x16x4_f64 %[c13], %[a11], %[b13], %[c13]\n\t" \
+  "s_waitcnt vmcnt(0)\n\t" \
+  "s_barrier\n\t" \
+  "v_mfma_f64_16x16x4_f64 %[c20], %[a12], %[b10], %[c20]\n\t" \
+  "ds_read_b64 %[a00], %[ard0] offset:0\n\t" \
+  "ds_read_b64 %[a01], %[ard0] offset:128\n\t" \
+  "v_mfma_f64_16x16x4_f64 %[c21], %[a12], %[b11], %[c21]\n\t" \
+  "ds_read_b64 %[a02], %[ard0] offset:256\n\t" \
+  "ds_read_b64 %[a03], %[ard0] offset:384\n\t" \
+  "v_mfma_f64_16x16x4_f64 %[c22], %[a12], %[b12], %[c22]\n\t" \
+  "ds_read_b64 %[b00], %[brd0] offset:0\n\t" \
+  "ds_read_b64 %[b01], %[brd0] offset:128\n\t" \
+  "v_mfma_f64_16x16x4_f64 %[c23], %[a12], %[b13], %[c23]\n\t" \
+  "ds_read_b64 %[b02], %[brd0] offset:256\n\t" \
+  "ds_read_b64 %[b03], %[brd0] offset:384\n\t" \
+  "v_mfma_f64_16x16x4_f64 %[c30], %[a13], %[b10], %[c30]\n\t" \
+  "v_mfma_f64_16x16x4_f64 %[c31], %[a13], %[b11], %[c31]\n\t" \
+  "v_mfma_f64_16x16x4_f64 %[c32], %[a13], %[b12], %[c32]\n\t" \
+  "v_mfma_f64_16x16x4_f64 %[c33], %[a13], %[b13], %[c33]\n\t" \
+  "s_sub_u32 %[cnt], %[cnt], 1\n\t" \
+  "s_cmp_lg_u32 %[cnt], 0\n\t" \
+  "s_cbranch_scc1 nk_tn8_loop_%=\n\t" \
+  "nk_tn8_after_%=:\n\t" \
+  "s_bitcmp1_b32 %[flags], 0\n\t" \
+  "s_cbranch_scc0 nk_tn8_even_%=\n\t" \
+  "s_waitcnt lgkmcnt(0)\n\t" \
+  "v_mfma_f64_16x16x4_f64 %[c00], %[a00], %[b00], %[c00]\n\t" \
+  "ds_read_b64 %[a10], %[ard0] offset:4608\n\t" \
+  "s_mov_b32 m0, %[dst1]\n\t" \
+  "s_nop 0\n\t" \
+  "global_load_lds_dwordx4 %[voa], s[92:93]\n\t" \
+  "v_mfma_f64_16x16x4_f64 %[c01], %[a00], %[b01], %[c01]\n\t" \
+  "ds_read_b64 %[a11], %[ard0] offset:4736\n\t" \
+  "s_add_u32 m0, m0, 9216\n\t" \
+  "s_add_u32 s92, s92, %[stra]\n\t" \
+  "s_addc_u32 s93, s93, 0\n\t" \
+  "v_mfma_f64_16x16x4_f64 %[c02], %[a00], %[b02], %[c02]\n\t" \
+  "ds_read_b64 %[a12], %[ard0] offset:4864\n\t" \
+  "global_load_lds_dwordx4 %[vob], s[94:95]\n\t" \
+  "s_sub_u32 m0, m0, 4608\n\t" \
+  "s_add_u32 s94, s94, %[strb]\n\t" \
+  "v_mfma_f64_16x16x4_f64 %[c03], %[a00], %[b03], %[c03]\n\t" \
+  "ds_read_b64 %[a13], %[ard0] offset:4992\n\t" \
+  "s_addc_u32 s95, s95, 0\n\t" \
+  "s_nop 0\n\t" \
+  "global_load_lds_dwordx4 %[voa], s[92:93]\n\t" \
+  "v_mfma_f64_16x16x4_f64 %[c10], %[a01], %[b00], %[c10]\n\t" \
+  "ds_read_b64 %[b10], %[brd0] offset:4608\n\t" \
+  "s_add_u32 m0, m0, 9216\n\t" \
+  "s_add_u32 s92, s92, %[stra]\n\t" \
+  "s_addc_u32 s93, s93, 0\n\t" \
+  "v_mfma_f64_16x16x4_f64 %[c11], %[a01], %[b01], %[c11]\n\t" \
+  "ds_read_b64 %[b11], %[brd0] offset:4736\n\t" \
+  "global_load_lds_dwordx4 %[vob], s[94:95]\n\t" \
+  "s_add_u32 s94, s94, %[strb]\n\t" \
+  "s_addc_u32 s95, s95, 0\n\t" \
+  "v_mfma_f64_16x16x4_f64 %[c12], %[a01], %[b02], %[c12]\n\t" \
+  "ds_read_b64 %[b12], %[brd0] offset:4864\n\t" \
+  "v_mfma_f64_16x16x4_f64 %[c13], %[a01], %[b03], %[c13]\n\t" \
+  "ds_read_b64 %[b13], %[brd0] offset:4992\n\t" \
+  "v_mfma_f64_16x16x4_f64 %[c20], %[a02], %[b00], %[c20]\n\t" \
+  "v_mfma_f64_16x16x4_f64 %[c21], %[a02], %[b01], %[c21]\n\t" \
+  "v_mfma_f64_16x16x4_f64 %[c22], %[a02], %[b02], %[c22]\n\t" \
+  "v_mfma_f64_16x16x4_f64 %[c23], %[a02], %[b03], %[c23]\n\t" \
+  "v_mfma_f64_16x16x4_f64 %[c30], %[a03], %[b00], %[c30]\n\t" \
+  "v_mfma_f64_16x16x4_f64 %[c31], %[a03], %[b01], %[c31]\n\t" \
+  "v_mfma_f64_16x16x4_f64 %[c32], %[a03], %[b02], %[c32]\n\t" \
+  "v_mfma_f64_16x16x4_f64 %[c33], %[a03], %[b03], %[c33]\n\t" \
+  "s_waitcnt lgkmcnt(0)\n\t" \
+  "v_mfma_f64_16x16x4_f64 %[c00], %[a10], %[b10], %[c00]\n\t" \
+  "v_mfma_f64_16x16x4_f64 %[c01], %[a10], %[b11], %[c01]\n\t" \
+  "v_mfma_f64_16x16x4_f64 %[c02], %[a10], %[b12], %[c02]\n\t" \
+  "v_mfma_f64_16x16x4_f64 %[c03], %[a10], %[b13], %[c03]\n\t" \
+  "v_mfma_f64_16x16x4_f64 %[c10], %[a11], %[b10], %[c10]\n\t" \
+  "v_mfma_f64_16x16x4_f64 %[c11], %[a11], %[b11], %[c11]\n\t" \
+  "v_mfma_f64_16x16x4_f64 %[c12], %[a11], %[b12], %[c12]\n\t" \
+  "v_mfma_f64_16x16x4_f64 %[c13], %[a11], %[b13], %[c13]\n\t" \
+  "s_waitcnt vmcnt(0)\n\t" \
+  "s_barrier\n\t" \
+  "v_mfma_f64_16x16x4_f64 %[c20], %[a12], %[b10], %[c20]\n\t" \
+  "ds_read_b64 %[a00], %[ard0] offset:18432\n\t" \
+  "ds_read_b64 %[a01], %[ard0] offset:18560\n\t" \
+  "v_mfma_f64_16x16x4_f64 %[c21], %[a12], %[b11], %[c21]\n\t" \
+  "ds_read_b64 %[a02], %[ard0] offset:18688\n\t" \
+  "ds_read_b64 %[a03], %[ard0] offset:18816\n\t" \
+  "v_mfma_f64_16x16x4_f64 %[c22], %[a12], %[b12], %[c22]\n\t" \
+  "ds_read_b64 %[b00], %[brd0] offset:18432\n\t" \
+  "ds_read_b64 %[b01], %[brd0] offset:18560\n\t" \
+  "v_mfma_f64_16x16x4_f64 %[c23], %[a12], %[b13], %[c23]\n\t" \
+  "ds_read_b64 %[b02], %[brd0] offset:18688\n\t" \
+  "ds_read_b64 %[b03], %[brd0] offset:18816\n\t" \
+  "v_mfma_f64_16x16x4_f64 %[c30], %[a13], %[b10], %[c30]\n\t" \
+  "v_mfma_f64_16x16x4_f64 %[c31], %[a13], %[b11], %[c31]\n\t" \
+  "v_mfma_f64_16x16x4_f64 %[c32], %[a13], %[b12], %[c32]\n\t" \
+  "v_mfma_f64_16x16x4_f64 %[c33], %[a13], %[b13], %[c33]\n\t" \
+  "s_bitcmp1_b32 %[flags], 1\n\t" \
+  "s_cbranch_scc0 nk_tn8_end_%=\n\t" \
+  "s_waitcnt lgkmcnt(0)\n\t" \
+  "v_mfma_f64_16x16x4_f64 %[c00], %[a00], %[b00], %[c00]\n\t" \
+  "ds_read_b64 %[a10], %[ard0] offset:23040\n\t" \
+  "v_mfma_f64_16x16x4_f64 %[c01], %[a00], %[b01], %[c01]\n\t" \
+  "ds_read_b64 %[a11], %[ard0] offset:23168\n\t" \
+  "v_mfma_f64_16x16x4_f64 %[c02], %[a00], %[b02], %[c02]\n\t" \
+  "ds_read_b64 %[a12], %[ard0] offset:23296\n\t" \
+  "v_mfma_f64_16x16x4_f64 %[c03], %[a00], %[b03], %[c03]\n\t" \
+  "ds_read_b64 %[a13], %[ard0] offset:23424\n\t" \
+  "v_mfma_f64_16x16x4_f64 %[c10], %[a01], %[b00], %[c10]\n\t" \
+  "ds_read_b64 %[b10], %[brd0] offset:23040\n\t" \
+  "v_mfma_f64_16x16x4_f64 %[c11], %[a01], %[b01], %[c11]\n\t" \
+  "ds_read_b64 %[b11], %[brd0] offset:23168\n\t" \
+  "v_mfma_f64_16x16x4_f64 %[c12], %[a01], %[b02], %[c12]\n\t" \
+  "ds_read_b64 %[b12], %[brd0] offset:23296\n\t" \
+  "v_mfma_f64_16x16x4_f64 %[c13], %[a01], %[b03], %[c13]\n\t" \
+  "ds_read_b64 %[b13], %[brd0] offset:23424\n\t" \
+  "v_mfma_f64_16x16x4_f64 %[c20], %[a02], %[b00], %[c20]\n\t" \
+  "v_mfma_f64_16x16x4_f64 %[c21], %[a02], %[b01], %[c21]\n\t" \
+  "v_mfma_f64_16x16x4_f64 %[c22], %[a02], %[b02], %[c22]\n\t" \
+  "v_mfma_f64_16x16x4_f64 %[c23], %[a02], %[b03], %[c23]\n\t" \
+  "v_mfma_f64_16x16x4_f64 %[c30], %[a03], %[b00], %[c30]\n\t" \
+  "v_mfma_f64_16x16x4_f64 %[c31], %[a03], %[b01], %[c31]\n\t" \
+  "v_mfma_f64_16x16x4_f64 %[c32], %[a03], %[b02], %[c32]\n\t" \
+  "v_mfma_f64_16x16x4_f64 %[c33], %[a03], %[b03], %[c33]\n\t" \
+  "s_waitcnt lgkmcnt(0)\n\t" \
+  "v_mfma_f64_16x16x4_f64 %[c00], %[a10], %[b10], %[c00]\n\t" \
+  "v_mfma_f64_16x16x4_f64 %[c01], %[a10], %[b11], %[c01]\n\t" \
+  "v_mfma_f64_16x16x4_f64 %[c02], %[a10], %[b12], %[c02]\n\t" \
+  "v_mfma_f64_16x16x4_f64 %[c03], %[a10], %[b13], %[c03]\n\t" \
+  "v_mfma_f64_16x16x4_f64 %[c10], %[a11], %[b10], %[c10]\n\t" \
+  "v_mfma_f64_16x16x4_f64 %[c11], %[a11], %[b11], %[c11]\n\t" \
+  "v_mfma_f64_16x16x4_f64 %[c12], %[a11], %[b12], %[c12]\n\t" \
+  "v_mfma_f64_16x16x4_f64 %[c13], %[a11], %[b13], %[c13]\n\t" \
+  "v_mfma_f64_16x16x4_f64 %[c20], %[a12], %[b10], %[c20]\n\t" \
+  "v_mfma_f64_16x16x4_f64 %[c21], %[a12], %[b11], %[c21]\n\t" \
+  "v_mfma_f64_16x16x4_f64 %[c22], %[a12], %[b12], %[c22]\n\t" \
+  "v_mfma_f64_16x16x4_f64 %[c23], %[a12], %[b13], %[c23]\n\t" \
+  "v_mfma_f64_16x16x4_f64 %[c30], %[a13], %[b10], %[c30]\n\t" \
+  "v_mfma_f64_16x16x4_f64 %[c31], %[a13], %[b11], %[c31]\n\t" \
+  "v_mfma_f64_16x16x4_f64 %[c32], %[a13], %[b12], %[c32]\n\t" \
+  "v_mfma_f64_16x16x4_f64 %[c33], %[a13], %[b13], %[c33]\n\t" \
+  "s_branch nk_tn8_end_%=\n\t" \
+  "nk_tn8_even_%=:\n\t" \
+  "s_bitcmp1_b32 %[flags], 1\n\t" \
+  "s_cbranch_scc0 nk_tn8_end_%=\n\t" \
+  "s_waitcnt lgkmcnt(0)\n\t" \
+  "v_mfma_f64_16x16x4_f64 %[c00], %[a00], %[b00], %[c00]\n\t" \
+  "ds_read_b64 %[a10], %[ard0] offset:4608\n\t" \
+  "v_mfma_f64_16x16x4_f64 %[c01], %[a00], %[b01], %[c01]\n\t" \
+  "ds_read_b64 %[a11], %[ard0] offset:4736\n\t" \
+  "v_mfma_f64_16x16x4_f64 %[c02], %[a00], %[b02], %[c02]\n\t" \
+  "ds_read_b64 %[a12], %[ard0] offset:4864\n\t" \
+  "v_mfma_f64_16x16x4_f64 %[c03], %[a00], %[b03], %[c03]\n\t" \
+  "ds_read_b64 %[a13], %[ard0] offset:4992\n\t" \
+  "v_mfma_f64_16x16x4_f64 %[c10], %[a01], %[b00], %[c10]\n\t" \
+  "ds_read_b64 %[b10], %[brd0] offset:4608\n\t" \
+  "v_mfma_f64_16x16x4_f64 %[c11], %[a01], %[b01], %[c11]\n\t" \
+  "ds_read_b64 %[b11], %[brd0] offset:4736\n\t" \
+  "v_mfma_f64_16x16x4_f64 %[c12], %[a01], %[b02], %[c12]\n\t" \
+  "ds_read_b64 %[b12], %[brd0] offset:4864\n\t" \
+  "v_mfma_f64_16x16x4_f64 %[c13], %[a01], %[b03], %[c13]\n\t" \
+  "ds_read_b64 %[b13], %[brd0] offset:4992\n\t" \
+  "v_mfma_f64_16x16x4_f64 %[c20], %[a02], %[b00], %[c20]\n\t" \
+  "v_mfma_f64_16x16x4_f64 %[c21], %[a02], %[b01], %[c21]\n\t" \
+  "v_mfma_f64_16x16x4_f64 %[c22], %[a02], %[b02], %[c22]\n\t" \
+  "v_mfma_f64_16x16x4_f64 %[c23], %[a02], %[b03], %[c23]\n\t" \
+  "v_mfma_f64_16x16x4_f64 %[c30], %[a03], %[b00], %[c30]\n\t" \
+  "v_mfma_f64_16x16x4_f64 %[c31], %[a03], %[b01], %[c31]\n\t" \
+  "v_mfma_f64_16x16x4_f64 %[c32], %[a03], %[b02], %[c32]\n\t" \
+  "v_mfma_f64_16x16x4_f64 %[c33], %[a03], %[b03], %[c33]\n\t" \
+  "s_waitcnt lgkmcnt(0)\n\t" \
+  "v_mfma_f64_16x16x4_f64 %[c00], %[a10], %[b10], %[c00]\n\t" \
+  "v_mfma_f64_16x16x4_f64 %[c01], %[a10], %[b11], %[c01]\n\t" \
+  "v_mfma_f64_16x16x4_f64 %[c02], %[a10], %[b12], %[c02]\n\t" \
+  "v_mfma_f64_16x16x4_f64 %[c03], %[a10], %[b13], %[c03]\n\t" \
+  "v_mfma_f64_16x16x4_f64 %[c10], %[a11], %[b10], %[c10]\n\t" \
+  "v_mfma_f64_16x16x4_f64 %[c11], %[a11], %[b11], %[c11]\n\t" \
+  "v_mfma_f64_16x16x4_f64 %[c12], %[a11], %[b12], %[c12]\n\t" \
+  "v_mfma_f64_16x16x4_f64 %[c13], %[a11], %[b13], %[c13]\n\t" \
+  "v_mfma_f64_16x16x4_f64 %[c20], %[a12], %[b10], %[c20]\n\t" \
+  "v_mfma_f64_16x16x4_f64 %[c21], %[a12], %[b11], %[c21]\n\t" \
+  "v_mfma_f64_16x16x4_f64 %[c22], %[a12], %[b12], %[c22]\n\t" \
+  "v_mfma_f64_16x16x4_f64 %[c23], %[a12], %[b13], %[c23]\n\t" \
+  "v_mfma_f64_16x16x4_f64 %[c30], %[a13], %[b10], %[c30]\n\t" \
+  "v_mfma_f64_16x16x4_f64 %[c31], %[a13], %[b11], %[c31]\n\t" \
+  "v_mfma_f64_16x16x4_f64 %[c32], %[a13], %[b12], %[c32]\n\t" \
+  "v_mfma_f64_16x16x4_f64 %[c33], %[a13], %[b13], %[c33]\n\t" \
+  "nk_tn8_end_%=:\n\t" \
+  ""
```

Measured after the change: 24.45. No clear change (-0.4%).
